# ubisoft/ubisoft-laforge-ZeroEGGS

Measured on AMD Instinct MI355X. Metric: train_frames_per_sec, higher is better.
Workload: dtype f32; 1 GPU; configs_v1.json nets (25.5M params, random-init), batch 32/GPU x 256-frame windows from synthetic 60fps 2-min clips, style example 384 frames, full train step (gather+fwd+loss+bwd+allreduce+RAdam); global_batch=32, window=256, parallelism=dp1

## Files before the change

### include/zeggs_hip.h

```cpp
#ifndef ZEGGS_HIP_H
#define ZEGGS_HIP_H
#include <stddef.h>
#include <stdint.h>

#ifdef __cplusplus
extern "C" {
#endif

int zeggs_version(void);
const char* zeggs_last_error(void);
int zeggs_set_option(const char* name, int value);
int zeggs_timing_ms(int which, float* ms);

int zeggs_gemm(const float* A, const float* B, float* C, const float* bias, int M, int N, int K,
               long sam, long sak, long sbk, long sbn, long scm, long scn, int nbatch, long bsA,
               long bsB, long bsC, float alpha, float beta, int act, void* stream);
int zeggs_gemm_tn_bias(const float* dy, long lddy, const float* x, long ldx, float* dW, long lddw, int M_contract, int N, int K,
                       float beta, float* db, void* stream);
int zeggs_gemm_direct_selftest(int big, int depth, int shield);
int zeggs_gemm_direct_state(int big, int depth, int shield);
int zeggs_gemm_direct_warm(void);
int zeggs_gemm_route(int direct, int shield, int depth, int reserve);
int zeggs_gemm_route_get(int* out4);
int zeggs_gemm_kbatch(const float* A, const float* B, float* C, int M, int N, int K, long sam, long sak, long sbk, long sbn,
// ... 68 lines not shown
                            const ZeggsStyleGrads*, void* ws, size_t ws_bytes, void* stream);
int zeggs_style_encoder_bwd_ex(const ZeggsStyleDims*, const ZeggsStyleParams*, const float* dout,
                               const ZeggsStyleGrads*, void* ws, size_t ws_bytes, void* stream, int grads_zeroed);
int zeggs_style_encoder_bwd_part(const ZeggsStyleDims*, const ZeggsStyleParams*, const float* dout, const ZeggsStyleGrads*, void* ws,
                                 size_t ws_bytes, void* stream, int grads_zeroed, int part);
typedef struct {
  int B, L, C, H, O;
} ZeggsStyleGruDims;
typedef struct {
  const float *c0_w, *c0_b;
  const float *c2_w, *c2_b;
  const float *w_ih, *w_hh, *b_ih, *b_hh;
  const float *w_ih_r, *w_hh_r, *b_ih_r, *b_hh_r;
  const float *p_w, *p_b;
} ZeggsStyleGruParams;
typedef struct {
  float *c0_w, *c0_b, *c2_w, *c2_b, *w_ih, *w_hh, *b_ih, *b_hh, *w_ih_r, *w_hh_r, *b_ih_r, *b_hh_r, *p_w, *p_b;
} ZeggsStyleGruGrads;
size_t zeggs_style_encoder_gru_workspace_bytes(const ZeggsStyleGruDims*);
int zeggs_style_encoder_gru_fwd(const ZeggsStyleGruDims*, const ZeggsStyleGruParams*, const float* x, float* out,
                                void* ws, size_t ws_bytes, void* stream);
int zeggs_style_encoder_gru_bwd(const ZeggsStyleGruDims*, const ZeggsStyleGruParams*, const float* dout,
                                const ZeggsStyleGruGrads*, void* ws, size_t ws_bytes, void* stream);
int zeggs_vae_reparam_fwd(const float* enc, const float* eps, float* z, float* mu_out ,
                          float* logvar_out , int B, int S, float temperature, void* stream);
int zeggs_vae_reparam_bwd(const float* enc, const float* eps, const float* dz, const float* dmu,
                          const float* dlogvar, float* denc, int B, int S, float temperature, void* stream);

typedef struct {
  int B, T, PI, PO, SP, ST, H;
  float dt;
  int film;
} ZeggsDecDims;
typedef struct {
  const float *l0_w, *l0_b;
  const float *w_ih0, *w_hh0, *b_ih0, *b_hh0;
  const float *w_ih1, *w_hh1, *b_ih1, *b_hh1;
  const float *l2_w, *l2_b;
  const float *c0_w, *c0_b, *c1_w, *c1_b, *c2_w, *c2_b;
  const float *l3_w, *l3_b;
  const float *g_w, *g_b, *be_w, *be_b;
} ZeggsDecParams;
typedef struct {
  float *l0_w, *l0_b, *w_ih0, *w_hh0, *b_ih0, *b_hh0, *w_ih1, *w_hh1, *b_ih1, *b_hh1, *l2_w, *l2_b, *c0_w,
      *c0_b, *c1_w, *c1_b, *c2_w, *c2_b, *l3_w, *l3_b, *g_w, *g_b, *be_w, *be_b;
} ZeggsDecGrads;
typedef struct {
  const float *in_mean, *in_std;
  const float *out_mean, *out_std;
} ZeggsDecStats;
size_t zeggs_decoder_workspace_bytes(const ZeggsDecDims*, int training);
int zeggs_decoder_fwd(const ZeggsDecDims*, const ZeggsDecParams*, const ZeggsDecStats*, const float* pose0,
                      const float* rpos0, const float* rrot0, const float* gaze, const float* speech,
                      const float* style, float* pose, float* rpos, float* rrot, int training, void* ws,
                      size_t ws_bytes, void* stream);
int zeggs_decoder_fwd_state(const ZeggsDecDims*, const ZeggsDecParams*, const ZeggsDecStats*, const float* pose0,
                            const float* rpos0, const float* rrot0, const float* gaze, const float* speech,
                            const float* style, float* pose, float* rpos, float* rrot, const float* h_in,
                            float* h_out, void* ws, size_t ws_bytes, void* stream);
int zeggs_persistent_state(int which );
int zeggs_tp_stamps(const ZeggsDecDims*, void* ws, size_t ws_bytes, unsigned long long* out );
int zeggs_tp_waits(const ZeggsDecDims*, void* ws, size_t ws_bytes, unsigned long long* out );
int zeggs_tp_dual_stamps(const ZeggsDecDims*, void* ws, size_t ws_bytes, unsigned long long* out );
int zeggs_bp_stamps(const ZeggsDecDims*, void* ws, size_t ws_bytes, unsigned long long* out );
int zeggs_bp_waits(const ZeggsDecDims*, void* ws, size_t ws_bytes, unsigned long long* out );
int zeggs_decoder_chain_errors(const ZeggsDecDims*, int training, void* ws, size_t ws_bytes, int* out);
int zeggs_decoder_chain_stamps(const ZeggsDecDims*, int training, void* ws, size_t ws_bytes,
                               unsigned long long* out );
int zeggs_decoder_bwd(const ZeggsDecDims*, const ZeggsDecParams*, const ZeggsDecStats*, const float* gaze,
                      const float* pose, const float* rpos, const float* rrot, const float* dpose,
                      const float* drpos, const float* drrot, const ZeggsDecGrads*, float* dspeech,
                      float* dstyle, void* ws, size_t ws_bytes, void* stream);
#define ZEGGS_STATUS_WORDS 4
#define ZEGGS_GAVE_UP_DECODE 1u
#define ZEGGS_GAVE_UP_TRAIN_FWD 2u
#define ZEGGS_GAVE_UP_BPTT 4u
#define ZEGGS_GAVE_UP_BATCH_FWD 8u
typedef struct {
  int prepared;
  int defer_wgrads;
  void* wgrad_stream;
  unsigned* status;
  int grads_zeroed;
} ZeggsDecCall;
int zeggs_decoder_fwd_ex(const ZeggsDecDims*, const ZeggsDecParams*, const ZeggsDecStats*, const float* pose0,
                         const float* rpos0, const float* rrot0, const float* gaze, const float* speech,
                         const float* style, float* pose, float* rpos, float* rrot, int training, void* ws,
                         size_t ws_bytes, void* stream, const ZeggsDecCall* call);
int zeggs_decoder_bwd_ex(const ZeggsDecDims*, const ZeggsDecParams*, const ZeggsDecStats*, const float* gaze,
                         const float* pose, const float* rpos, const float* rrot, const float* dpose,
                         const float* drpos, const float* drrot, const ZeggsDecGrads*, float* dspeech,
                         float* dstyle, void* ws, size_t ws_bytes, void* stream, const ZeggsDecCall* call);
int zeggs_decoder_fwd_state_ex(const ZeggsDecDims*, const ZeggsDecParams*, const ZeggsDecStats*, const float* pose0,
                               const float* rpos0, const float* rrot0, const float* gaze, const float* speech,
                               const float* style, float* pose, float* rpos, float* rrot, const float* h_in,
                               float* h_out, void* ws, size_t ws_bytes, void* stream, const ZeggsDecCall* call);
size_t zeggs_decoder_batch_workspace_bytes(const ZeggsDecDims*);
int zeggs_decoder_batch_prepare(const ZeggsDecDims*, const ZeggsDecParams*, const ZeggsDecStats*, void* ws, size_t ws_bytes,
                                void* stream);
int zeggs_decoder_state_init(const ZeggsDecDims*, const ZeggsDecParams*, const ZeggsDecStats*, const float* pose0,
                             const float* rpos0, const float* rrot0, const float* gaze0, const float* style0, float* h_out,
                             void* ws, size_t ws_bytes, void* stream);
int zeggs_decoder_fwd_batch(const ZeggsDecDims*, const ZeggsDecParams*, const ZeggsDecStats*, const float* pose0,
                            const float* rpos0, const float* rrot0, const float* gaze, const float* speech,
                            const float* style, float* pose, float* rpos, float* rrot, const float* h_in, float* h_out,
                            void* ws, size_t ws_bytes, void* stream, const ZeggsDecCall* call, int mode);
int zeggs_decoder_batch_last_path(void);
int zeggs_decoder_wgrads(const ZeggsDecDims*, const ZeggsDecGrads*, void* ws, size_t ws_bytes, int what, void* stream);
int zeggs_decoder_prepare(const ZeggsDecDims*, const ZeggsDecParams*, const ZeggsDecStats*, void* ws, size_t ws_bytes,
                          void* stream);
int zeggs_side_stream(void** out );

typedef struct {
  int B, T, J, S;
  float dt;
} ZeggsLossDims;
size_t zeggs_loss_workspace_bytes(const ZeggsLossDims*);
int zeggs_loss_fwd_bwd(const ZeggsLossDims*, const int* parents, const float* o_pose, const float* o_rpos,
                       const float* o_rrot, const float* w_pose, const float* w_rpos, const float* w_rrot,
                       const float* gaze, const float* mu, const float* logvar, float kl_weight, float* terms,
                       float* dpose, float* drpos, float* drrot, float* dmu, float* dlogvar, float gscale,
                       void* ws, size_t ws_bytes, void* stream);

int zeggs_loss_prepare_truth(const ZeggsLossDims*, const int* parents, const float* w_pose, const float* w_rpos,
                             const float* w_rrot, const float* gaze, void* ws, size_t ws_bytes, void* stream);
int zeggs_loss_fwd_bwd_ex(const ZeggsLossDims*, const int* parents, const float* o_pose, const float* o_rpos,
                          const float* o_rrot, const float* w_pose, const float* w_rpos, const float* w_rrot,
                          const float* gaze, const float* mu, const float* logvar, float kl_weight, float* terms,
                          float* dpose, float* drpos, float* drrot, float* dmu, float* dlogvar, float gscale,
                          void* ws, size_t ws_bytes, void* stream, int truth_prepared);

#define ZEGGS_EVAL_COLS 22
size_t zeggs_loss_eval_workspace_bytes(const ZeggsLossDims*);
int zeggs_loss_eval(const ZeggsLossDims*, const int* parents, const float* o_pose, const float* o_rpos, const float* o_rrot,
                    const float* w_pose, const float* w_rpos, const float* w_rrot, const float* gaze, const float* mu,
                    const float* logvar, double* rows , void* ws, size_t ws_bytes, void* stream);
int zeggs_eval_accumulate(const double* rows, const int* group , int B, int groups, double* acc, void* stream);
int zeggs_gemm_fixed_order(int on);
enum {
  ZEGGS_GEMM_ROUTE_NONE = 0,
  ZEGGS_GEMM_ROUTE_SKINNY,
  ZEGGS_GEMM_ROUTE_M32_SPLIT,
  ZEGGS_GEMM_ROUTE_M32,
  ZEGGS_GEMM_ROUTE_MID_SPLIT,
  ZEGGS_GEMM_ROUTE_SK_DIRECT,
  ZEGGS_GEMM_ROUTE_SK_BF16_SPLIT,
  ZEGGS_GEMM_ROUTE_SK_DMA,
  ZEGGS_GEMM_ROUTE_SK_LDS_128,
  ZEGGS_GEMM_ROUTE_SK_LDS_256,
  ZEGGS_GEMM_ROUTE_SPLITK,
  ZEGGS_GEMM_ROUTE_HALF,
  ZEGGS_GEMM_ROUTE_TILE_128,
  ZEGGS_GEMM_ROUTE_TILE_64,
  ZEGGS_GEMM_ROUTE_COUNT
};
int zeggs_test_gemm_route_log(int reset, int* last4, long* counts, int ncounts);

int zeggs_radam_step(float* p, const float* g, float* m, float* v, long n, float beta1, float beta2, float eps,
                     float step_scale, int rectified, void* stream);
int zeggs_radam_step_guarded(float* p, const float* g, float* m, float* v, long n, float beta1, float beta2, float eps,
                             float step_scale, int rectified, unsigned* status, const float* gflag, void* stream);
int zeggs_radam_step_guarded_part(float* p, const float* g, float* m, float* v, long n, float beta1, float beta2, float eps,
                                  float step_scale, int rectified, unsigned* status, const float* gflag, int count_skip,
                                  void* stream);
int zeggs_radam_step_wd(float* p, const float* g, float* m, float* v, long n, float beta1, float beta2, float eps,
                        float step_scale, int rectified, float decay, unsigned* status, const float* gflag, int count_skip,
                        void* stream);
int zeggs_radam_step_c(float* p, const float* g, float* m, float* v, long n, float beta1, float beta2, float comp1, float comp2,
                       float eps, float step_scale, int rectified, float decay, unsigned* status, const float* gflag,
                       int count_skip, void* stream);
int zeggs_radam_step_d(float* p, const float* g, float* m, float* v, long n, double beta1, double beta2, double comp1, double comp2,
                       float eps, float step_scale, int rectified, float decay, unsigned* status, const float* gflag,
                       int count_skip, void* stream);
int zeggs_status_flag(const unsigned* status, float* dst , void* stream);
int zeggs_test_cotenant(int workgroups, int threads, float ms, float* scratch, long n, void* stream);
int zeggs_test_attention_fwd(const float* qkv, float* O, float* lse, int B, int L, int E, int NH, float p, uint64_t seed, void* stream);
int zeggs_test_attention_bwd(const float* qkv, const float* O, const float* lse, const float* dO, float* dqkv, float* dsum,
                             float* dbias , int B, int L, int E, int NH, float p, uint64_t seed, void* stream);

int zeggs_gather_windows(const float* frames, int width, const int64_t* starts, int B, int T, float* out,
                         void* stream);
int zeggs_gather_rows(const float* frames, int width, const int64_t* rows, long nrows, float* out, int out_ld,
                      void* stream);

typedef struct {
  int n_fft, hop, n_mels, fs;
  float fps, min_clip;
  double pre_emph;
  int flags;
} ZeggsMelDims;
long zeggs_mel_stft_frames(const ZeggsMelDims*, long n_samples);
size_t zeggs_mel_workspace_bytes(const ZeggsMelDims*, long n_samples);
int zeggs_mel_features(const ZeggsMelDims*, const float* wav, long n_samples, const double* filterbank,
                       int n_frames, float* out, void* ws, size_t ws_bytes, void* stream);
long zeggs_mel_frames_ready(const ZeggsMelDims*, long n_samples);
size_t zeggs_mel_range_workspace_bytes(const ZeggsMelDims*, long k0, long k1);
int zeggs_mel_features_range(const ZeggsMelDims*, const float* wav, long n_samples, int final, const double* filterbank,
                             long k0, long k1, float* out, void* ws, size_t ws_bytes, void* stream);
long zeggs_mel_window_first_sample(const ZeggsMelDims*, long k0);
int zeggs_mel_features_window(const ZeggsMelDims*, const float* wav_window, long base, long n_samples, int final,
                              const double* filterbank, long k0, long k1, float* out, void* ws, size_t ws_bytes, void* stream);
int zeggs_mel_last_form(void);

size_t zeggs_loudness_workspace_bytes(long n_samples, int nblocks, long chunk);
int zeggs_loudness_gain(const float* wav, long n_samples, int rate, double target, const double* coef, const double* trans,
                        long chunk, const long* blk_lo, const long* blk_hi, int nblocks, int f32_stages, double* result,
                        float* gain32, void* ws, size_t ws_bytes, void* stream);

int zeggs_gather_example(const float* frames, int width, const int64_t* rows, int B, int L, const float* mean, const float* stdv,
                         float* out, int out_width, int pad, void* stream);
int zeggs_normalize_rows(float* x, long rows, int width, long ld, const float* mean, const float* stdv,
                         float std_scalar, void* stream);

int zeggs_fill(float* dst, long n, float value, void* stream);
int zeggs_scale_copy(float* dst, const float* src, long n, const float* dev_scale ,
                     float alpha, void* stream);
int zeggs_randn(float* out, long n, uint64_t seed, void* stream);
int zeggs_dropout(float* x, long n, float p, uint64_t seed, void* stream);
int zeggs_broadcast_time(float* out , const float* z , int B, int T, int S, void* stream);
int zeggs_sum_time(float* dz , const float* dout , int B, int T, int S, void* stream);

int zeggs_normalize_vec_fwd(const float* x, float* y, long rows, int width, float eps, void* stream);
int zeggs_normalize_vec_bwd(const float* x, const float* dy, float* dx, long rows, int width, float eps, void* stream);
int zeggs_vectorize_input_fwd(int B, int J, const float* root_pos, const float* root_rot, const float* root_vel,
                              const float* root_vrt, const float* lpos, const float* ltxy, const float* lvel,
                              const float* lvrt, const float* gaze_pos, const float* in_mean, const float* in_std,
                              float* out, void* stream);
int zeggs_vectorize_input_bwd(int B, int J, const float* root_pos, const float* root_rot, const float* gaze_pos,
                              const float* in_std, const float* dout, float* d_root_pos, float* d_root_rot,
                              float* d_root_vel, float* d_root_vrt, float* d_lpos, float* d_ltxy, float* d_lvel,
                              float* d_lvrt, float* d_gaze_pos, void* stream);
int zeggs_devectorize_output_fwd(int B, int J, float dt, const float* predicted, const float* root_pos,
                                 const float* root_rot, const float* out_mean, const float* out_std, float* pose,
                                 float* new_root_pos, float* new_root_rot, void* stream);
int zeggs_devectorize_output_bwd(int B, int J, float dt, const float* predicted, const float* root_pos,
                                 const float* root_rot, const float* out_mean, const float* out_std, const float* d_pose,
                                 const float* d_new_root_pos, const float* d_new_root_rot, float* d_predicted,
                                 float* d_root_pos, float* d_root_rot, void* stream);
int zeggs_kl_div_fwd(const float* mu, const float* logvar, int B, int S, float* out, void* stream);
int zeggs_kl_div_bwd(const float* mu, const float* logvar, int B, int S, const float* dout, float* dmu, float* dlogvar,
                     void* stream);
int zeggs_mask_from_lengths(const int64_t* lengths, int B, int max_len, uint8_t* mask, void* stream);

typedef struct {
  int N, J, hips, spine2, head;
  double dt;
  int order;
} ZeggsAnimDims;
typedef struct {
  double *root_pos, *root_rot, *root_vel, *root_vrt;
  double *lpos, *lrot, *lvel, *lvrt;
  float* ltxy;
  double *cpos, *crot, *cvel, *cvrt;
  float* ctxy;
  double *gaze_pos, *gaze_dir;
} ZeggsAnimOut;
size_t zeggs_anim_features_workspace_bytes(const ZeggsAnimDims*);
int zeggs_anim_features(const ZeggsAnimDims*, const int* parents, const double* euler_deg, const double* positions,
                        const ZeggsAnimOut* out, void* ws, size_t ws_bytes, void* stream);

typedef struct {
  int T, J, rebase;
  double start_pos[3], start_rot[4];
  int order;
} ZeggsBvhDims;
int zeggs_pose_to_bvh(const ZeggsBvhDims*, const float* root_pos, const float* root_rot, const float* lpos,
                      const float* ltxy, double* positions, double* euler_deg, void* stream);

int zeggs_pose_to_bvh_table(const ZeggsBvhDims*, const float* root_pos, const float* root_rot, const float* lpos,
                            const float* ltxy, const float* ref_root_pos, const float* ref_root_rot, const int* seq,
                            double* table, void* stream);

int zeggs_write_table_text(const char* path, int append, const double* table , long rows, int cols);
int zeggs_parse_table_text(const char* text, size_t len, double* table , long rows, int cols);
int zeggs_format_table_text(const double* table , long rows, int cols, char* out, size_t cap, size_t* written);

size_t zeggs_table_text_workspace_bytes(long rows, int cols);
int zeggs_table_text_device(const double* table, long rows, int cols, char* text, size_t cap, long long* row_end,
                            unsigned* status, void* ws, size_t ws_bytes, void* stream);

int zeggs_spline_chunk(int* chunk, int* halo, int* narrow_width);
size_t zeggs_spline_resample_workspace_bytes(long N, int W);
int zeggs_spline_resample(const double* y, long N, int W, long M, double* out, void* ws, size_t ws_bytes, void* stream);
size_t zeggs_rot_stretch_workspace_bytes(long N, int J, long M);
int zeggs_rot_stretch(const double* euler_deg, long N, int J, long M, int order, double* out_deg, void* ws, size_t ws_bytes, void* stream);
int zeggs_audio_prepare(const float* wav, long n_wav, const long* intervals, int n_intervals, long start, long end, float* out_f32,
                        double* out_f64, void* stream);
int zeggs_center_take(double* positions, double* euler_deg, long N, int J, int order, int round_f32, void* ws, size_t ws_bytes,
                      void* stream);
size_t zeggs_masked_stats_workspace_bytes(long R, int D);
int zeggs_masked_stats(const float* x, const unsigned char* mask, long R, int D, double* mean, double* std_, double* pooled, void* ws,
                       size_t ws_bytes, void* stream);

int zeggs_sweep_graph_stats(long* captures, long* replays);

#ifdef __cplusplus
}
#endif
#endif
```

### ubisoft-laforge-zeroeggs_amd/csrc/encoders.hip

```cpp
#include "../../include/zeggs_hip.h"
#include "common.h"
#include "gemm.h"
#include "kernels.h"

namespace {

struct SpeechWs {
  float *h0p, *h1, *wf1, *wb1;
  float *d2, *dh1pp, *dh0p, *dh0, *dwf1;
};

SpeechWs carve_speech(const ZeggsSpeechDims& d, Arena& a) {
  SpeechWs w;
  const long BT = (long)d.B * d.T, pad = d.KW - 1;
  w.h0p = a.f((long)d.B * (d.T + pad) * d.H);
  w.h1 = a.f(BT * d.O);
  w.wf1 = a.f((long)d.KW * d.H * d.O);
  w.wb1 = a.f((long)d.KW * d.O * d.H);
  w.d2 = a.f(BT * d.O);
  w.dh1pp = a.f((long)d.B * (d.T + 2 * pad) * d.O);
  w.dh0p = a.f((long)d.B * (d.T + pad) * d.H);
  w.dh0 = a.f(BT * d.H);
  w.dwf1 = a.f((long)d.KW * d.H * d.O);
  return w;
// ... 130 lines not shown
  w.lse = w.dsum = nullptr;
  if (w.fused) {
    w.P = w.Pd = nullptr;
    w.lse = a.f(B * NH * L); w.dsum = a.f(B * NH * L);
  } else {
    w.P = a.f(B * NH * L * L);
    w.Pd = d.dropout ? a.f(B * NH * L * L) : nullptr;
  }
  w.O = a.f(BL * E);
  w.ao = a.f(BL * E); w.ma = a.f(BL); w.ra = a.f(BL);
  w.ap = a.f(B * LP * E);
  w.f1p = a.f(B * LP * E);
  w.f2 = a.f(BL * E); w.mf = a.f(BL); w.rf = a.f(BL);
  w.f = a.f(BL * E);
  w.S = w.fused ? nullptr : a.f(B * NH * L * L);
  long big = BL * (long)(H > 3 * E ? H : 3 * E);
  const long HE = H > E ? H : E;
  long dw = (long)C * H;
  if ((long)H * E > dw) dw = (long)H * E;
  if ((long)E * E > dw) dw = (long)E * E;
  w.t0 = a.f(B * LP * HE); w.t1 = a.f(big); w.t2 = a.f(big); w.t3 = a.f(B * LP * HE);
  w.dqkv = a.f(BL * 3 * E);
  w.dwf = a.f(3L * dw);
  w.t0a = a.f(B * LP * E); w.t0b = a.f(B * LP * E); w.t1a = a.f(BL * E);
  return w;
}

}

extern "C" size_t zeggs_style_encoder_workspace_bytes(const ZeggsStyleDims* d) {
  Arena a(nullptr, 0);
  carve_style(*d, a);
  return a.off + 256;
}

extern "C" int zeggs_style_encoder_fwd(const ZeggsStyleDims* dp, const ZeggsStyleParams* P, const float* x,
                                       const float* pos, float* out, void* ws, size_t ws_bytes, void* stream) {
  return zeggs_style_encoder_fwd_part(dp, P, x, pos, out, ws, ws_bytes, stream, 3);
}
extern "C" size_t zeggs_style_encoder_input_offset(const ZeggsStyleDims* d) {
  char base[1];
  Arena a(base, ~(size_t)0);
  StyleWs w = carve_style(*d, a);
  return (size_t)((char*)w.xp - base);
}
extern "C" int zeggs_style_encoder_fwd_part(const ZeggsStyleDims* dp, const ZeggsStyleParams* P, const float* x, const float* pos,
                                            float* out, void* ws, size_t ws_bytes, void* stream, int part) {
  const ZeggsStyleDims& d = *dp;
  hipStream_t s = (hipStream_t)stream;
  Arena a(ws, ws_bytes);
  StyleWs w = carve_style(d, a);
  ZCHECK(a.ok(), "style encoder: workspace too small (%zu < %zu)", ws_bytes, a.off);
  ZCHECK(d.E % d.NH == 0, "style encoder: E %% heads != 0");
  const int B = d.B, L = d.L, C = d.C, H = d.H, E = d.E, NH = d.NH, HD = E / NH, LP = L + 2;
  const long BL = (long)B * L;
  const float p2 = d.dropout ? 0.2f : 0.f, p1 = d.dropout ? 0.1f : 0.f;
  const float eps = 1e-5f;
  const bool fuse0 = H <= 512, fuse = E <= 512;
  const RowView c1v = rv(w.c1, L, (long)LP * H), c2v = rv(w.c2, L, (long)LP * E);
  if (part & 1) {
  {
    const PackConvW items[4] = {{w.wf0, nullptr, P->c0_w, H, C, 3}, {w.wf4, w.wb4, P->c4_w, E, H, 3},
                                {w.wff0, w.wfb0, P->ff0_w, E, E, 3}, {w.wff2, w.wfb2, P->ff2_w, E, E, 3}};
    ZTRY(k_pack_conv_w_multi(items, 4, s));
  }
  if (!(part & 4)) ZTRY(k_pad_rows(w.xp, x, B, L, C, 1, 1, 0, s));
  if (fuse0) ZTRY(conv_flat(w.xp, C, w.wf0, 3 * C, H, w.c1, B * LP - 2, s));
  else ZTRY(conv_gemm(w.xp, (long)LP * C, C, w.wf0, 3 * C, H, w.c1, H, (long)LP * H, P->c0_b, B, L, ACT_RELU, s));
  }
  if (!(part & 2)) return 0;
  if (fuse0) {
    LnFwdFused q = ln_fwd_fused_args((int)BL, H, eps);
    q.x = c1v; q.pre_bias = P->c0_b; q.pre_act = ACT_RELU;
    q.y = rv(w.a1p + H, L, (long)LP * H); q.gamma = P->ln0_g; q.beta = P->ln0_b; q.mean = w.m1; q.rstd = w.r1;
    q.p_post = p2; q.seed_post = d.seed + 1; q.pad_L = L;
    ZTRY(k_ln_fwd_fused(q, s));
  } else {
  ZTRY(k_layernorm_fwd_v(rv(w.a1p + H, L, (long)LP * H), c1v, rv(nullptr), P->ln0_g, P->ln0_b, w.m1, w.r1,
                          (int)BL, H, eps, s));
  ZTRY(k_dropout_rows(w.a1p + H, (int)BL, H, H, L, (long)LP * H, p2, d.seed + 1, s));
  ZTRY(k_pad_edges(w.a1p, B, L, H, 1, 1, 0, s));
  }
  if (fuse) ZTRY(conv_flat(w.a1p, H, w.wf4, 3 * H, E, w.c2, B * LP - 2, s));
  else ZTRY(conv_gemm(w.a1p, (long)LP * H, H, w.wf4, 3 * H, E, w.c2, E, (long)LP * E, P->c4_b, B, L, ACT_RELU, s));
  if (fuse) {
    LnFwdFused q = ln_fwd_fused_args((int)BL, E, eps);
    q.x = c2v; q.pre_bias = P->c4_b; q.pre_act = ACT_RELU;
    q.y = rv(w.h); q.gamma = P->ln1_g; q.beta = P->ln1_b; q.mean = w.m2; q.rstd = w.r2;
    q.p_post = p2; q.seed_post = d.seed + 2; q.table = pos; q.table_L = L;
    ZTRY(k_ln_fwd_fused(q, s));
  } else {
  ZTRY(k_layernorm_fwd_v(rv(w.h), c2v, rv(nullptr), P->ln1_g, P->ln1_b, w.m2, w.r2, (int)BL, E, eps, s));
  ZTRY(k_dropout(w.h, BL * E, p2, d.seed + 2, s));
  ZTRY(k_add_rows_bcast(w.h, pos, B, L, E, s));
  }
  ZTRY(gemm_nt(w.h, E, P->in_w, E, w.qkv, 3 * E, P->in_b, (int)BL, 3 * E, E, ACT_NONE, 0.f, s));
  if (w.fused) {
    ZTRY(k_attn_fwd(w.qkv, w.O, w.lse, B, L, E, NH, p1, d.seed + 3, s));
  } else {
  {
    GemmArgs g = gemm_args(w.qkv, w.qkv + E, w.S, L, L, HD);
    g.sam = 3 * E; g.sak = 1; g.sbk = 1; g.sbn = 3 * E; g.scm = L; g.scn = 1;
    g.nb1 = NH; g.bsA0 = (long)L * 3 * E; g.bsA1 = HD; g.bsB0 = (long)L * 3 * E; g.bsB1 = HD;
    g.bsC0 = (long)NH * L * L; g.bsC1 = (long)L * L; g.alpha = 1.0f / sqrtf((float)HD);
    ZTRY(launch_gemm(g, B * NH, s));
  }
  ZTRY(k_softmax_fwd(w.P, w.Pd, w.S, (long)B * NH * L, L, p1, d.seed + 3, s));
  {
    const float* Pm = w.Pd ? w.Pd : w.P;
    GemmArgs g = gemm_args(Pm, w.qkv + 2 * E, w.O, L, HD, L);
    g.sam = L; g.sak = 1; g.sbk = 3 * E; g.sbn = 1; g.scm = E; g.scn = 1;
    g.nb1 = NH; g.bsA0 = (long)NH * L * L; g.bsA1 = (long)L * L; g.bsB0 = (long)L * 3 * E; g.bsB1 = HD;
    g.bsC0 = (long)L * E; g.bsC1 = HD;
    ZTRY(launch_gemm(g, B * NH, s));
  }
  }
  ZTRY(gemm_nt(w.O, E, P->out_w, E, w.ao, E, P->out_b, (int)BL, E, E, ACT_NONE, 0.f, s));
  if (fuse) {
    LnFwdFused q = ln_fwd_fused_args((int)BL, E, eps);
    q.x = rv(w.ao); q.res = rv(w.h); q.y = rv(w.ap + E, L, (long)LP * E); q.gamma = P->lna_g; q.beta = P->lna_b;
    q.mean = w.ma; q.rstd = w.ra; q.p_pre = p1; q.seed_pre = d.seed + 4; q.pad_L = L;
    ZTRY(k_ln_fwd_fused(q, s));
  } else {
  ZTRY(k_dropout(w.ao, BL * E, p1, d.seed + 4, s));
  ZTRY(k_layernorm_fwd_v(rv(w.ap + E, L, (long)LP * E), rv(w.ao), rv(w.h), P->lna_g, P->lna_b, w.ma, w.ra, (int)BL, E,
                          eps, s));
  ZTRY(k_pad_edges(w.ap, B, L, E, 1, 1, 0, s));
  }
  ZTRY(conv_gemm(w.ap, (long)LP * E, E, w.wff0, 3 * E, E, w.f1p + E, E, (long)LP * E, P->ff0_b, B, L, ACT_RELU, s));
  ZTRY(k_pad_edges(w.f1p, B, L, E, 1, 1, 0, s));
  ZTRY(conv_gemm(w.f1p, (long)LP * E, E, w.wff2, 3 * E, E, w.f2, E, (long)L * E, fuse ? nullptr : P->ff2_b, B, L, ACT_NONE, s));
  if (fuse) {
    LnFwdFused q = ln_fwd_fused_args((int)BL, E, eps);
    q.x = rv(w.f2); q.pre_bias = P->ff2_b; q.pre_act = ACT_NONE; q.res = rv(w.ap + E, L, (long)LP * E); q.y = rv(w.f); q.gamma = P->lnf_g; q.beta = P->lnf_b;
    q.mean = w.mf; q.rstd = w.rf; q.p_pre = p1; q.seed_pre = d.seed + 5;
    ZTRY(k_ln_fwd_fused(q, s));
  } else {
  ZTRY(k_dropout(w.f2, BL * E, p1, d.seed + 5, s));
  ZTRY(k_layernorm_fwd_v(rv(w.f), rv(w.f2), rv(w.ap + E, L, (long)LP * E), P->lnf_g, P->lnf_b, w.mf, w.rf, (int)BL, E,
                          eps, s));
  }
  ZTRY(k_meanpool_fwd(out, w.f, B, L, E, s));
  return 0;
}

extern "C" int zeggs_style_encoder_bwd(const ZeggsStyleDims* dp, const ZeggsStyleParams* P, const float* dout,
                                       const ZeggsStyleGrads* G, void* ws, size_t ws_bytes, void* stream) {
  return zeggs_style_encoder_bwd_ex(dp, P, dout, G, ws, ws_bytes, stream, 0);
}
extern "C" int zeggs_style_encoder_bwd_ex(const ZeggsStyleDims* dp, const ZeggsStyleParams* P, const float* dout,
                                          const ZeggsStyleGrads* G, void* ws, size_t ws_bytes, void* stream, int grads_zeroed) {
  return zeggs_style_encoder_bwd_part(dp, P, dout, G, ws, ws_bytes, stream, grads_zeroed, 3);
}
extern "C" int zeggs_style_encoder_bwd_part(const ZeggsStyleDims* dp, const ZeggsStyleParams* P, const float* dout,
                                            const ZeggsStyleGrads* G, void* ws, size_t ws_bytes, void* stream, int grads_zeroed,
                                            int part) {
  ZCHECK(part >= 1 && part <= 3, "style encoder bwd: part must be 1, 2 or 3");
  const bool chain = part & 1, inl = part == 3, only_w = part == 2;
  const ZeggsStyleDims& d = *dp;
  const float gb = grads_zeroed ? 1.f : 0.f;
  hipStream_t s = (hipStream_t)stream;
  Arena a(ws, ws_bytes);
  StyleWs w = carve_style(d, a);
  ZCHECK(a.ok(), "style encoder bwd: workspace too small");
  const int B = d.B, L = d.L, C = d.C, H = d.H, E = d.E, NH = d.NH, HD = E / NH, LP = L + 2;
  const long BL = (long)B * L;
  const float p2 = d.dropout ? 0.2f : 0.f, p1 = d.dropout ? 0.1f : 0.f;
  float *t0 = w.t0, *t1 = w.t1, *t2 = w.t2, *t3 = w.t3;
  float *t0a = w.t0a, *t0b = w.t0b, *t1a = w.t1a;
  auto dw_ff2 = [&](hipStream_t q) -> int {
    ZTRY(conv_dw_gemm(w.f1p, (long)LP * E, E, t0a + E, E, (long)LP * E, w.dwf, 3 * E, E, B, L, q));
    return k_unpack_conv_dw(G->ff2_w, w.dwf, E, E, 3, q);
  };
  auto dw_ff0 = [&](hipStream_t q) -> int {
    ZTRY(conv_dw_gemm(w.ap, (long)LP * E, E, t0b + E, E, (long)LP * E, w.dwf, 3 * E, E, B, L, q));
    return k_unpack_conv_dw(G->ff0_w, w.dwf, E, E, 3, q);
  };
  auto dw_out = [&](hipStream_t q) -> int { return gemm_tn(t1a, E, w.O, E, G->out_w, E, (int)BL, E, E, gb, q); };
  auto dw_in = [&](hipStream_t q) -> int { return gemm_tn(w.dqkv, 3 * E, w.h, E, G->in_w, E, (int)BL, 3 * E, E, gb, q); };
  auto dw_c4 = [&](hipStream_t q) -> int {
    ZTRY(conv_dw_gemm(w.a1p, (long)LP * H, H, t0 + E, E, (long)LP * E, w.dwf, 3 * H, E, B, L, q));
    return k_unpack_conv_dw(G->c4_w, w.dwf, E, H, 3, q);
  };
  auto dw_c0 = [&](hipStream_t q) -> int {
    ZTRY(conv_dw_gemm(w.xp, (long)LP * C, C, t2, H, (long)L * H, w.dwf, 3 * C, H, B, L, q));
    return k_unpack_conv_dw(G->c0_w, w.dwf, H, C, 3, q);
  };
  if (only_w) {
    ZTRY(dw_ff2(s)); ZTRY(dw_ff0(s)); ZTRY(dw_out(s)); ZTRY(dw_in(s)); ZTRY(dw_c4(s)); ZTRY(dw_c0(s));
    return 0;
  }
  (void)chain;
  if (!grads_zeroed) {
    ZTRY(k_fill(G->lnf_g, E, 0.f, s)); ZTRY(k_fill(G->lnf_b, E, 0.f, s)); ZTRY(k_fill(G->ff2_b, E, 0.f, s));
    ZTRY(k_fill(G->ff0_b, E, 0.f, s)); ZTRY(k_fill(G->lna_g, E, 0.f, s)); ZTRY(k_fill(G->lna_b, E, 0.f, s));
    ZTRY(k_fill(G->out_b, E, 0.f, s)); ZTRY(k_fill(G->ln1_g, E, 0.f, s)); ZTRY(k_fill(G->ln1_b, E, 0.f, s));
    ZTRY(k_fill(G->c4_b, E, 0.f, s)); ZTRY(k_fill(G->ln0_g, H, 0.f, s)); ZTRY(k_fill(G->ln0_b, H, 0.f, s));
    ZTRY(k_fill(G->c0_b, H, 0.f, s));
    if (w.fused) ZTRY(k_fill(G->in_b, 3 * E, 0.f, s));
  }
  const RowView t0in = rv(t0 + E, L, (long)LP * E);
  const RowView t0ain = rv(t0a + E, L, (long)LP * E), t0bin = rv(t0b + E, L, (long)LP * E);
  {
    LnBwdFused q = ln_bwd_fused_args((int)BL, E);
    q.dy_pool = dout; q.pool_L = L;
    q.x = rv(w.f2); q.res = rv(w.ap + E, L, (long)LP * E); q.gamma = P->lnf_g; q.mean = w.mf; q.rstd = w.rf;
    q.dgamma = G->lnf_g; q.dbeta = G->lnf_b;
    q.dx_raw = rv(t2); q.out = t0ain; q.pad_L = L; q.p_post = p1; q.seed_post = d.seed + 5; q.dbias = G->ff2_b;
    ZTRY(k_ln_bwd_fused(q, s));
  }
  if (inl) ZTRY(dw_ff2(s));
  ZTRY(conv_gemm(t0a, (long)LP * E, E, w.wfb2, 3 * E, E, t1, E, (long)L * E, nullptr, B, L, ACT_NONE, s));
  {
    LnBwdFused q = ln_bwd_fused_args((int)BL, E);
    q.dyA = rv(t1); q.out = t0bin; q.pad_L = L; q.ysave = rv(w.f1p + E, L, (long)LP * E); q.act = ACT_RELU; q.dbias = G->ff0_b;
    ZTRY(k_ln_bwd_fused(q, s));
  }
  if (inl) ZTRY(dw_ff0(s));
  ZTRY(conv_gemm(t0b, (long)LP * E, E, w.wfb0, 3 * E, E, t1, E, (long)L * E, nullptr, B, L, ACT_NONE, s));
  {
    LnBwdFused q = ln_bwd_fused_args((int)BL, E);
    q.dyA = rv(t2); q.dyB = rv(t1);
    q.x = rv(w.ao); q.res = rv(w.h); q.gamma = P->lna_g; q.mean = w.ma; q.rstd = w.ra; q.dgamma = G->lna_g; q.dbeta = G->lna_b;
    q.dx_raw = rv(t3); q.out = rv(t1a); q.p_post = p1; q.seed_post = d.seed + 4; q.dbias = G->out_b;
    ZTRY(k_ln_bwd_fused(q, s));
  }
  if (inl) ZTRY(dw_out(s));
  ZTRY(gemm_nn(t1a, E, P->out_w, E, t2, E, (int)BL, E, E, 0.f, s));
  if (w.fused) {
    ZTRY(k_attn_bwd(w.qkv, w.O, w.lse, t2, w.dqkv, w.dsum, G->in_b, B, L, E, NH, p1, d.seed + 3, s));
  } else {
  const float* Pm = w.Pd ? w.Pd : w.P;
  {
    GemmArgs g = gemm_args(t2, w.qkv + 2 * E, w.S, L, L, HD);
    g.sam = E; g.sak = 1; g.sbk = 1; g.sbn = 3 * E; g.scm = L; g.scn = 1;
    g.nb1 = NH; g.bsA0 = (long)L * E; g.bsA1 = HD; g.bsB0 = (long)L * 3 * E; g.bsB1 = HD;
    g.bsC0 = (long)NH * L * L; g.bsC1 = (long)L * L;
    ZTRY(launch_gemm(g, B * NH, s));
  }
  {
    GemmArgs g = gemm_args(Pm, t2, w.dqkv + 2 * E, L, HD, L);
    g.sam = 1; g.sak = L; g.sbk = E; g.sbn = 1; g.scm = 3 * E; g.scn = 1;
    g.nb1 = NH; g.bsA0 = (long)NH * L * L; g.bsA1 = (long)L * L; g.bsB0 = (long)L * E; g.bsB1 = HD;
    g.bsC0 = (long)L * 3 * E; g.bsC1 = HD;
    ZTRY(launch_gemm(g, B * NH, s));
  }
  ZTRY(k_softmax_bwd(w.S, w.S, w.P, (long)B * NH * L, L, p1, d.seed + 3, s));
  const float sc = 1.0f / sqrtf((float)HD);
  {
    GemmArgs g = gemm_args(w.S, w.qkv + E, w.dqkv, L, HD, L);
    g.sam = L; g.sak = 1; g.sbk = 3 * E; g.sbn = 1; g.scm = 3 * E; g.scn = 1;
    g.nb1 = NH; g.bsA0 = (long)NH * L * L; g.bsA1 = (long)L * L; g.bsB0 = (long)L * 3 * E; g.bsB1 = HD;
    g.bsC0 = (long)L * 3 * E; g.bsC1 = HD; g.alpha = sc;
    ZTRY(launch_gemm(g, B * NH, s));
  }
  {
    GemmArgs g = gemm_args(w.S, w.qkv, w.dqkv + E, L, HD, L);
    g.sam = 1; g.sak = L; g.sbk = 3 * E; g.sbn = 1; g.scm = 3 * E; g.scn = 1;
    g.nb1 = NH; g.bsA0 = (long)NH * L * L; g.bsA1 = (long)L * L; g.bsB0 = (long)L * 3 * E; g.bsB1 = HD;
    g.bsC0 = (long)L * 3 * E; g.bsC1 = HD; g.alpha = sc;
    ZTRY(launch_gemm(g, B * NH, s));
  }
  }
  if (inl) ZTRY(dw_in(s));
  if (!w.fused) ZTRY(k_colsum(G->in_b, w.dqkv, BL, 3 * E, 3 * E, gb, s));
  ZTRY(gemm_nn(w.dqkv, 3 * E, P->in_w, E, t1, E, (int)BL, 3 * E, E, 0.f, s));
  {
    LnBwdFused q = ln_bwd_fused_args((int)BL, E);
    q.dyA = rv(t1); q.dyB = rv(t3); q.p_pre = p2; q.seed_pre = d.seed + 2;
    q.x = rv(w.c2, L, (long)LP * E); q.gamma = P->ln1_g; q.mean = w.m2; q.rstd = w.r2; q.dgamma = G->ln1_g; q.dbeta = G->ln1_b;
    q.out = t0in; q.pad_L = L; q.ysave = rv(w.c2, L, (long)LP * E); q.act = ACT_RELU; q.dbias = G->c4_b;
    ZTRY(k_ln_bwd_fused(q, s));
  }
  if (inl) ZTRY(dw_c4(s));
  ZTRY(conv_gemm(t0, (long)LP * E, E, w.wb4, 3 * E, H, t1, H, (long)L * H, nullptr, B, L, ACT_NONE, s));
  {
    LnBwdFused q = ln_bwd_fused_args((int)BL, H);
    q.dyA = rv(t1); q.p_pre = p2; q.seed_pre = d.seed + 1;
    q.x = rv(w.c1, L, (long)LP * H); q.gamma = P->ln0_g; q.mean = w.m1; q.rstd = w.r1; q.dgamma = G->ln0_g; q.dbeta = G->ln0_b;
    q.out = rv(t2); q.ysave = rv(w.c1, L, (long)LP * H); q.act = ACT_RELU; q.dbias = G->c0_b;
    ZTRY(k_ln_bwd_fused(q, s));
  }
  if (inl) ZTRY(dw_c0(s));
  return 0;
}
```

### ubisoft-laforge-zeroeggs_amd/csrc/gemm.h

```cpp
#pragma once
#include <hip/hip_runtime.h>

struct GemmArgs {
  const float* A;
  const float* B;
  float* C;
  const float* bias;
  int M, N, K;
  long sam, sak, sbk, sbn, scm, scn;
  long bsA0, bsA1, bsB0, bsB1, bsC0, bsC1;
  int nb1;
  int kbatch;
  long kbsA, kbsB;
  int splitk;
  float alpha, beta;
  int act;
  float* asum;
};

GemmArgs gemm_args(const float* A, const float* B, float* C, int M, int N, int K);
int launch_gemm(GemmArgs g, int nbatch, hipStream_t s, bool* asum_taken = nullptr);
int gemm_nt(const float* x, long ldx, const float* W, long ldw, float* y, long ldy, const float* bias, int M,
            int N, int K, int act, float beta, hipStream_t s);
struct GemmNtItem { const float* x; long ldx; const float* W; long ldw; float* y; long ldy; const float* bias; int N, K, act; };
int gemm_nt_multi(const GemmNtItem* items, int n, int M, hipStream_t s);
int gemm_nn(const float* dy, long lddy, const float* W, long ldw, float* dx, long lddx, int M, int N_contract,
            int K_out, float beta, hipStream_t s);
int gemm_nn_actbwd(const float* dy, long lddy, const float* W, long ldw, float* dx, long lddx, int M, int N_contract,
                   int K_out, float beta, const float* ysave, long ldys, int act, hipStream_t s);
int gemm_tn(const float* dy, long lddy, const float* x, long ldx, float* dW, long lddw, int M_contract, int N,
            int K, float beta, hipStream_t s);
int gemm_tn_bias(const float* dy, long lddy, const float* x, long ldx, float* dW, long lddw, int M_contract, int N,
                 int K, float beta, float* db, hipStream_t s);
```

### ubisoft-laforge-zeroeggs_amd/csrc/gemm.hip

```cpp
#include <type_traits>
#include "common.h"
#include <vector>

#include "gemm.h"
#include "gemm_route.h"
#include "kernels.h"

extern int g_gemm_split_bf16;
bool gemm_split_ok(const GemmArgs& g);
int launch_tn_split(GemmArgs g, hipStream_t s);
bool stream_capturing(hipStream_t s);

int g_gemm_streamk_wgs = 0;
int g_gemm_wg_target = 6144;

namespace {

constexpr int BK = 16;

template <int E>
__device__ __forceinline__ void load_contig(float (&r)[E], const float* p, int nvalid) {
  if (nvalid >= E) {
    if constexpr (E == 16) {
#pragma unroll
// ... 394 lines not shown
    int mo[MT], no[NT];
#pragma unroll
    for (int i = 0; i < MT; ++i) { const int m = m_base + 32 * i + l31; mo[i] = m < g.M ? m : g.M - 1; }
#pragma unroll
    for (int j = 0; j < NT; ++j) { const int n = n_base + 32 * j + l31; no[j] = n < g.N ? n : g.N - 1; }
    unsigned voa[MT], vob[NT];
#pragma unroll
    for (int i = 0; i < MT; ++i) voa[i] = (unsigned)(((long)mo[i] + (long)kh * g.sak) * 4);
#pragma unroll
    for (int j = 0; j < NT; ++j) vob[j] = (unsigned)(((long)no[j] + (long)kh * g.sbk) * 4);
    f16v acc[MT][NT];
#pragma unroll
    for (int i = 0; i < MT; ++i)
#pragma unroll
      for (int j = 0; j < NT; ++j)
#pragma unroll
        for (int e = 0; e < 16; ++e) acc[i][j][e] = 0.f;
    float sa[MT];
#pragma unroll
    for (int i = 0; i < MT; ++i) sa[i] = 0.f;
    int c = c0;
    while (c < c1) {
      const int kb = c / chunks_per_batch, cb = c - kb * chunks_per_batch;
      int ce = c1 - kb * chunks_per_batch;
      ce = ce < chunks_per_batch ? ce : chunks_per_batch;
      const int p0 = cb * CH, p1 = ce * CH < npairs ? ce * CH : npairs, n = p1 - p0;
      const float* Ab = g.A + (long)kb * g.kbsA + (long)(2 * p0) * g.sak;
      const float* Bb = g.B + (long)kb * g.kbsB + (long)(2 * p0) * g.sbk;
      const long a2 = 2 * g.sak, b2 = 2 * g.sbk;
      float ra[D][MT], rb[D][NT];
      auto fetch = [&](int slot, int pair) {
        const unsigned long long ap = (unsigned long long)(Ab + (long)pair * a2), bp = (unsigned long long)(Bb + (long)pair * b2);
        const unsigned alo = __builtin_amdgcn_readfirstlane((unsigned)ap), ahi = __builtin_amdgcn_readfirstlane((unsigned)(ap >> 32));
        const unsigned blo = __builtin_amdgcn_readfirstlane((unsigned)bp), bhi = __builtin_amdgcn_readfirstlane((unsigned)(bp >> 32));
        const unsigned long long as = ((unsigned long long)ahi << 32) | alo, bs = ((unsigned long long)bhi << 32) | blo;
#pragma unroll
        for (int i = 0; i < MT; ++i) asm volatile("global_load_dword %0, %1, %2" : "=v"(ra[slot][i]) : "v"(voa[i]), "s"(as) : "memory");
#pragma unroll
        for (int j = 0; j < NT; ++j) asm volatile("global_load_dword %0, %1, %2" : "=v"(rb[slot][j]) : "v"(vob[j]), "s"(bs) : "memory");
      };
#define ZG_LANDED(S, Y)                                                                                                       \
  do {                                                                                                                         \
    if constexpr (MT == 4)                                                                                                     \
      asm volatile("s_waitcnt vmcnt(%10)\n\tv_add_f32 %6, %6, %0\n\tv_add_f32 %7, %7, %1\n\tv_add_f32 %8, %8, %2\n\tv_add_f32 %9, %9, %3" \
                   : "+v"(ra[S][0]), "+v"(ra[S][1]), "+v"(ra[S][MT > 2 ? 2 : 0]), "+v"(ra[S][MT > 3 ? 3 : 1]),              \
                     "+v"(rb[S][0]), "+v"(rb[S][1]), "+v"(sa[0]), "+v"(sa[1]), "+v"(sa[MT > 2 ? 2 : 0]), "+v"(sa[MT > 3 ? 3 : 1]) \
                   : "n"(Y) : "memory");                                                                                       \
    else                                                                                                                       \
      asm volatile("s_waitcnt vmcnt(%6)\n\tv_add_f32 %4, %4, %0\n\tv_add_f32 %5, %5, %1"                                       \
                   : "+v"(ra[S][0]), "+v"(ra[S][1]), "+v"(rb[S][0]), "+v"(rb[S][1]), "+v"(sa[0]), "+v"(sa[1]) : "n"(Y) : "memory"); \
  } while (0)
      static_assert((MT == 4 || MT == 2) && NT == 2, "direct kernel: wave tiles 128 x 64 and 64 x 64");
      constexpr int LG = MT + NT;
      auto mma = [&](int slot) {
#pragma unroll
        for (int i = 0; i < MT; ++i)
#pragma unroll
          for (int j = 0; j < NT; ++j) acc[i][j] = __builtin_amdgcn_mfma_f32_32x32x2f32(ra[slot][i], rb[slot][j], acc[i][j], 0, 0, 0);
      };
#pragma unroll
      for (int u = 0; u < D; ++u)
        if (u < n) fetch(u, u);
      int p = 0;
      for (; p + 2 * D <= n; p += D) {
#pragma unroll
        for (int u = 0; u < D; ++u) {
          ZG_LANDED(u, (D - 1) * LG);
          mma(u);
          __builtin_amdgcn_sched_barrier(0);
          fetch(u, p + u + D);
          __builtin_amdgcn_sched_barrier(0);
        }
      }
#pragma unroll
      for (int u = 0; u < D; ++u)
        if (p + u < n) ZG_LANDED(u, 0);
#pragma unroll
      for (int u = 0; u < D; ++u)
        if (p + u < n) {
          mma(u);
          if (p + u + D < n) { fetch(u, p + u + D); ZG_LANDED(u, 0); }
        }
      p += D;
#pragma unroll
      for (int u = 0; u < D; ++u)
        if (p + u < n) mma(u);
#undef ZG_LANDED
      c = (kb + 1) * chunks_per_batch < c1 ? (kb + 1) * chunks_per_batch : c1;
    }
#pragma unroll
    for (int i = 0; i < MT; ++i)
#pragma unroll
      for (int j = 0; j < NT; ++j) {
        const int nn = n_base + 32 * j + l31;
        if (nn >= g.N) continue;
#pragma unroll
        for (int e = 0; e < 16; ++e) {
          const int m = m_base + 32 * i + (e & 3) + 8 * (e >> 2) + 4 * kh;
          if (m < g.M) atomicAdd(g.C + (long)m * g.scm + nn, g.alpha * acc[i][j][e]);
        }
      }
    if (g.asum != nullptr && (tile % width) / gsz == 0 && wn == 0) {
#pragma unroll
      for (int i = 0; i < MT; ++i) {
        const float v = sa[i] + __shfl_xor(sa[i], 32, 64);
        const int m = m_base + 32 * i + l31;
        if (kh == 0 && m < g.M) atomicAdd(g.asum + m, g.alpha * v);
      }
    }
    it += c1 - c0;
  }
}
template <int MT, int NT, int D>
__global__ __launch_bounds__(256, 2) void gemm_tn_direct_kernel(GemmArgs g, int tiles_x, int tiles_y, int chunks_per_batch) {
  tn_direct_body<MT, NT, D>(g, tiles_x, tiles_y, chunks_per_batch);
}
template <int MT, int NT, int D>
__global__ __launch_bounds__(256, 1) void gemm_tn_direct_shield_kernel(GemmArgs g, int tiles_x, int tiles_y, int chunks_per_batch) {
  asm volatile("" ::: "v255", "a255");
  tn_direct_body<MT, NT, D>(g, tiles_x, tiles_y, chunks_per_batch);
}
int g_gemm_direct = 1;
int g_gemm_direct_depth = 4;
int g_gemm_direct_shield = 0;
int g_gemm_asum = 1;
int g_gemm_direct_reserve = 0;
int g_gemm_direct_wgs = 0;
static thread_local int tl_route[4] = {-1, -1, -1, -1};
static DirectFirstUse g_direct_first_use;
static TnRoute tn_route() {
  return resolve(tl_route, TnRoute{g_gemm_direct, g_gemm_direct_shield, g_gemm_direct_depth, g_gemm_direct_reserve},
                 g_direct_first_use.disabled.load(std::memory_order_acquire));
}
static TnShape tn_shape(const GemmArgs& g) { return TnShape{g.M, g.N, g.K, g.kbatch, g.sak, g.sbk, g.sam, g.sbn, g.scn}; }
static int device_cus() {
  int dev = 0, ncu = 256;
  if (hipGetDevice(&dev) == hipSuccess) (void)hipDeviceGetAttribute(&ncu, hipDeviceAttributeMultiprocessorCount, dev);
  return ncu;
}
int launch_tn_direct(const GemmArgs& g, const DirectPlan& p, hipStream_t s) {
#define ZG_DIRECT(MT_, D_)                                                                                                    \
  do {                                                                                                                         \
    if (p.shield) hipLaunchKernelGGL((gemm_tn_direct_shield_kernel<MT_, 2, D_>), dim3((unsigned)p.nwg), dim3(256), 0, s, g, p.tx, p.ty, p.cpb); \
    else hipLaunchKernelGGL((gemm_tn_direct_kernel<MT_, 2, D_>), dim3((unsigned)p.nwg), dim3(256), 0, s, g, p.tx, p.ty, p.cpb); \
  } while (0)
  if (p.big) { if (p.depth == 8) ZG_DIRECT(4, 8); else if (p.depth == 6) ZG_DIRECT(4, 6); else ZG_DIRECT(4, 4); }
  else { if (p.depth == 8) ZG_DIRECT(2, 8); else if (p.depth == 6) ZG_DIRECT(2, 6); else ZG_DIRECT(2, 4); }
#undef ZG_DIRECT
  ZLAUNCH_CHECK("gemm_tn_direct");
  return 0;
}

enum GemmRoute { GR_NONE = 0, GR_SKINNY, GR_M32_SPLIT, GR_M32, GR_MID_SPLIT, GR_SK_DIRECT, GR_SK_BF16_SPLIT, GR_SK_DMA, GR_SK_LDS_128,
                 GR_SK_LDS_256, GR_SPLITK, GR_HALF, GR_TILE_128, GR_TILE_64, GR_COUNT };
struct GemmRouteLog { int route, splitk, bm, bn; long count[GR_COUNT]; };
static thread_local GemmRouteLog tl_gemm_log;
static inline void log_route(int route, int splitk, int bm, int bn) {
  tl_gemm_log.route = route; tl_gemm_log.splitk = splitk; tl_gemm_log.bm = bm; tl_gemm_log.bn = bn;
  ++tl_gemm_log.count[route];
}
template <int BM, int BN, int WM, int WN>
int launch_streamk_cfg(GemmArgs g, int ncu, hipStream_t s) {
  const int tx = cdiv(g.N, BN), ty = cdiv(g.M, BM);
  const int kt = cdiv(g.K, BK) * g.kbatch;
  g.splitk = kt;
  constexpr int resident = WM * WN > 4 ? 2 : GEMM_MINB;
  long nwg = (long)ncu * (g_gemm_streamk_wgs > 0 ? g_gemm_streamk_wgs : resident);
  const long total = (long)tx * ty * kt;
  if (nwg > total / 16) nwg = total / 16 > 0 ? total / 16 : 1;
  dim3 grid((unsigned)nwg), block(WM * WN * 64);
  const bool akc = (g.sak == 1), bkc = (g.sbk == 1) && (g.sbn != 1 || g.N == 1);
  if (!akc && g.sam != 1) { zeggs_set_error("gemm: A has no unit stride (sam=%ld sak=%ld)", g.sam, g.sak); return -1; }
  if (!bkc && g.sbn != 1) { zeggs_set_error("gemm: B has no unit stride (sbk=%ld sbn=%ld)", g.sbk, g.sbn); return -1; }
  if (akc && bkc) hipLaunchKernelGGL((gemm_streamk_kernel<BM, BN, WM, WN, true, true>), grid, block, 0, s, g, tx, ty);
  else if (akc && !bkc) hipLaunchKernelGGL((gemm_streamk_kernel<BM, BN, WM, WN, true, false>), grid, block, 0, s, g, tx, ty);
  else if (!akc && bkc) hipLaunchKernelGGL((gemm_streamk_kernel<BM, BN, WM, WN, false, true>), grid, block, 0, s, g, tx, ty);
  else hipLaunchKernelGGL((gemm_streamk_kernel<BM, BN, WM, WN, false, false>), grid, block, 0, s, g, tx, ty);
  ZLAUNCH_CHECK("gemm_streamk");
  return 0;
}
static DirectCheck direct_selftest(const DirectPlan& variant) {
  const bool big = variant.big, shield = variant.shield;
  const int M = big ? 64 * 4 * 2 + 37 : 64 * 2 * 2 + 21, N = 128 + 27, K = 2 * 173;
  const long ldA = M + 3, ldB = N + 5;
  std::vector<float> hA((size_t)K * ldA), hB((size_t)K * ldB), hC((size_t)M * N + M);
  unsigned lcg = 12345u;
  auto rnd = [&]() { lcg = lcg * 1664525u + 1013904223u; return (float)((int)(lcg >> 9) - (1 << 22)) * (1.f / (1 << 22)); };
  for (auto& v : hA) v = rnd();
  for (auto& v : hB) v = rnd();
  hipStream_t st = nullptr;
  float* dA = nullptr;
  auto run = [&]() {
    ZCHECK(hipStreamCreateWithFlags(&st, hipStreamNonBlocking) == hipSuccess, "direct TN GEMM self-test: no stream");
    ZCHECK(hipMalloc(&dA, (hA.size() + hB.size() + hC.size()) * 4) == hipSuccess, "direct TN GEMM self-test: no memory");
    float *dB = dA + hA.size(), *dC = dB + hB.size();
    ZCHECK(hipMemcpyAsync(dA, hA.data(), hA.size() * 4, hipMemcpyHostToDevice, st) == hipSuccess &&
           hipMemcpyAsync(dB, hB.data(), hB.size() * 4, hipMemcpyHostToDevice, st) == hipSuccess &&
           hipMemsetAsync(dC, 0, hC.size() * 4, st) == hipSuccess, "direct TN GEMM self-test: copy failed");
    GemmArgs g = gemm_args(dA, dB, dC, M, N, K);
    g.sam = 1; g.sak = ldA; g.sbk = ldB; g.sbn = 1; g.scm = N; g.scn = 1; g.asum = dC + (size_t)M * N;
    ZTRY(launch_tn_direct(g, direct_grid(variant, tn_shape(g), device_cus(), g_gemm_direct_wgs, 0), st));
    ZCHECK(hipMemcpyAsync(hC.data(), dC, hC.size() * 4, hipMemcpyDeviceToHost, st) == hipSuccess &&
           hipStreamSynchronize(st) == hipSuccess, "direct TN GEMM self-test: copy back failed");
    return 0;
  };
  const bool ran = run() == 0;
  if (dA) (void)hipFree(dA);
  if (st) (void)hipStreamDestroy(st);
  if (!ran) return DirectCheck::UNAVAILABLE;
  const float* hS = hC.data() + (size_t)M * N;
  double worst = 0.0;
  for (int m = 0; m < M; ++m) {
    double sa = 0.0;
    for (int k = 0; k < K; ++k) sa += hA[(size_t)k * ldA + m];
    worst = fmax(worst, fabs(sa - hS[m]));
  }
  for (int m = 0; m < M; m += 3)
    for (int n = 0; n < N; ++n) {
      double acc = 0.0;
      for (int k = 0; k < K; ++k) acc += (double)hA[(size_t)k * ldA + m] * hB[(size_t)k * ldB + n];
      worst = fmax(worst, fabs(acc - hC[(size_t)m * N + n]));
    }
  if (worst < 2e-3) return DirectCheck::AGREES;
  fprintf(stderr, "zeggs: direct TN GEMM self-test (wave tile %s, depth %d%s) is off by %.3g\n", big ? "128x64" : "64x64",
          variant.depth, shield ? ", shield" : "", worst);
  return DirectCheck::MISMATCH;
}
int launch_streamk(GemmArgs g, hipStream_t s, bool* asum_taken) {
  if (gemm_split_ok(g)) { log_route(GR_SK_BF16_SPLIT, 0, 256, 128); return launch_tn_split(g, s); }
  const int ncu = device_cus();
  const DirectPlan plan = direct_plan(tn_route(), tn_shape(g), ncu, g_gemm_direct_wgs);
  if (plan.use && g_direct_first_use.go(plan, [s] { return stream_capturing(s); }, direct_selftest)) {
    if (asum_taken) *asum_taken = g.asum != nullptr;
    log_route(GR_SK_DIRECT, 0, plan.big ? 256 : 128, 128);
    return launch_tn_direct(g, plan, s);
  }
  if (dma_ok(g)) { log_route(GR_SK_DMA, 0, 128, 128); return launch_tn_dma(g, s); }
  if (tn_big_output(g.M, g.N) && g.M >= 512) { log_route(GR_SK_LDS_256, 0, 256, 128); return launch_streamk_cfg<256, 128, 4, 2>(g, ncu, s); }
  log_route(GR_SK_LDS_128, 0, 128, 128);
  return launch_streamk_cfg<128, 128, 2, 2>(g, ncu, s);
}

struct SkinnyArgs {
  const float *x, *W, *bias;
  float* y;
  const float* ysave;
  long ldx, ldw, ldy, ldys;
  int M, N, K, act;
  float beta;
};
template <int NBM, bool WKC>
__device__ __forceinline__ void skinny_body(const SkinnyArgs& a, int bx) {
  __shared__ f4 red[8][NBM][64];
  const int tid = threadIdx.x, lane = tid & 63, wave = tid >> 6, r = lane & 15, g = lane >> 4;
  const int M = a.M, N = a.N, K = a.K;
  const int n0 = bx * 16, nblk = (K + 15) >> 4;
  const int wcol = n0 + r < N ? n0 + r : N - 1;
  const float* wp = WKC ? a.W + (long)wcol * a.ldw + 4 * g : a.W + (long)(4 * g) * a.ldw + wcol;
  const float* xp[NBM];
#pragma unroll
  for (int nb = 0; nb < NBM; ++nb) { const int row = nb * 16 + r; xp[nb] = a.x + (long)(row < M ? row : M - 1) * a.ldx + 4 * g; }
  f4 acc[NBM];
#pragma unroll
  for (int nb = 0; nb < NBM; ++nb) acc[nb] = f4{0.f, 0.f, 0.f, 0.f};
  constexpr int GR = 4;
  float wa[GR][4], xa[GR][NBM][4], wq[GR][4], xq[GR][NBM][4];
  auto load = [&](float (&w)[GR][4], float (&xv)[GR][NBM][4], int i0) {
#pragma unroll
    for (int u = 0; u < GR; ++u) {
      const int kb = wave + 8 * (i0 + u);
      const int nv = kb < nblk ? K - (kb * 16 + 4 * g) : 0;
      if constexpr (WKC) load_contig<4>(w[u], wp + kb * 16, nv);
      else {
#pragma unroll
        for (int j = 0; j < 4; ++j) w[u][j] = j < nv ? wp[(long)(kb * 16 + j) * a.ldw] : 0.f;
      }
#pragma unroll
      for (int nb = 0; nb < NBM; ++nb) load_contig<4>(xv[u][nb], xp[nb] + kb * 16, nv);
    }
  };
  auto comp = [&](const float (&w)[GR][4], const float (&xv)[GR][NBM][4]) {
#pragma unroll
    for (int u = 0; u < GR; ++u)
#pragma unroll
      for (int j = 0; j < 4; ++j)
#pragma unroll
        for (int nb = 0; nb < NBM; ++nb) acc[nb] = __builtin_amdgcn_mfma_f32_16x16x4f32(xv[u][nb][j], w[u][j], acc[nb], 0, 0, 0);
  };
  const int ni = (nblk - wave + 7) / 8;
  load(wa, xa, 0);
  for (int i = 0; i < ni; i += 2 * GR) {
    if (i + GR < ni) load(wq, xq, i + GR);
    comp(wa, xa);
    if (i + 2 * GR < ni) load(wa, xa, i + 2 * GR);
    if (i + GR < ni) comp(wq, xq);
  }
#pragma unroll
  for (int nb = 0; nb < NBM; ++nb) red[wave][nb][lane] = acc[nb];
  __syncthreads();
  if (tid < NBM * 64) {
    const int nb = tid >> 6, l = tid & 63;
    f4 sum = red[0][nb][l];
#pragma unroll
    for (int w = 1; w < 8; ++w) sum += red[w][nb][l];
    const int col = n0 + (l & 15);
    if (col < N) {
      const float bv = a.bias ? a.bias[col] : 0.f;
#pragma unroll
      for (int q = 0; q < 4; ++q) {
        const int row = nb * 16 + 4 * (l >> 4) + q;
        if (row < M) {
          float* yp = a.y + (long)row * a.ldy + col;
          float v = sum[q] + bv;
          if (a.beta != 0.f) v += a.beta * *yp;
          if (a.ysave) {
            const float ys = a.ysave[(long)row * a.ldys + col];
            v = a.act == ACT_ELU ? v * d_elu_grad_from_out(ys) : a.act == ACT_RELU ? (ys > 0.f ? v : 0.f) : v;
          } else v = d_act(v, a.act);
          *yp = v;
        }
      }
    }
  }
}
template <int NBM, bool WKC>
__global__ __launch_bounds__(512) void skinny_k(SkinnyArgs a) {
  skinny_body<NBM, WKC>(a, blockIdx.x);
}
struct SkinnyMulti { SkinnyArgs p[3]; int nb[3]; };
template <int NBM, bool WKC>
__global__ __launch_bounds__(512) void skinny_multi_k(SkinnyMulti m) {
  int bx = blockIdx.x;
  if (bx < m.nb[0]) { skinny_body<NBM, WKC>(m.p[0], bx); return; }
  bx -= m.nb[0];
  if (bx < m.nb[1]) { skinny_body<NBM, WKC>(m.p[1], bx); return; }
  skinny_body<NBM, WKC>(m.p[2], bx - m.nb[1]);
}

int launch_skinny(const SkinnyArgs& a, bool wkc, hipStream_t s) {
  const int nbm = cdiv(a.M, 16);
  dim3 grid(cdiv(a.N, 16)), block(512);
#define ZEGGS_SKINNY(NB)                                                             \
  do {                                                                               \
    if (wkc) hipLaunchKernelGGL((skinny_k<NB, true>), grid, block, 0, s, a);         \
    else hipLaunchKernelGGL((skinny_k<NB, false>), grid, block, 0, s, a);            \
  } while (0)
  if (nbm == 1) ZEGGS_SKINNY(1);
  else if (nbm == 2) ZEGGS_SKINNY(2);
  else if (nbm == 3) ZEGGS_SKINNY(3);
  else ZEGGS_SKINNY(4);
#undef ZEGGS_SKINNY
  ZLAUNCH_CHECK("gemm_skinny");
  return 0;
}
bool skinny_ok(const GemmArgs& g, int nbatch) {
  return g.M <= 64 && nbatch == 1 && g.kbatch == 1 && g.sak == 1 && g.scn == 1 && g.alpha == 1.f && g.N >= 64 && g.K >= 64 &&
         ((g.sbk == 1 && g.sbn != 1) || g.sbn == 1) && (g.beta == 0.f || (g.bias == nullptr && g.act == ACT_NONE));
}
SkinnyArgs skinny_args(const GemmArgs& g) {
  SkinnyArgs a;
  memset(&a, 0, sizeof(a));
  a.x = g.A; a.ldx = g.sam; a.W = g.B; a.y = g.C; a.ldy = g.scm; a.bias = g.bias; a.M = g.M; a.N = g.N; a.K = g.K;
  a.act = g.act; a.beta = g.beta;
  a.ldw = (g.sbk == 1 && g.sbn != 1) ? g.sbn : g.sbk;
  return a;
}

}

void zeggs_gemm_set_dma(int on) { g_gemm_dma = on; }
void zeggs_gemm_set_direct(int mode, int wgs) { if (mode >= 0) g_gemm_direct = mode; if (wgs >= 0) g_gemm_direct_wgs = wgs; }
void zeggs_gemm_set_direct_depth(int d) { g_gemm_direct_depth = d; }
void zeggs_gemm_set_direct_shield(int on) { g_gemm_direct_shield = on; }
void zeggs_gemm_set_direct_reserve(int n) { g_gemm_direct_reserve = n; }
extern "C" int zeggs_gemm_route(int direct, int shield, int depth, int reserve) {
  const int r[4] = {direct, shield, depth, reserve};
  memcpy(tl_route, r, sizeof(r));
  return 0;
}
extern "C" int zeggs_gemm_route_get(int* out4) {
  const TnRoute r = tn_route();
  out4[0] = r.direct; out4[1] = r.shield; out4[2] = r.depth; out4[3] = r.reserve;
  return 0;
}
void zeggs_gemm_set_asum(int on) { g_gemm_asum = on; }
int g_gemm_skinny = 1;
int g_gemm_streamk = 1;
int g_gemm_mid_split = 1;
static thread_local int t_gemm_fixed_order = 0;
extern "C" int zeggs_gemm_fixed_order(int on) {
  const int prev = t_gemm_fixed_order;
  t_gemm_fixed_order = on != 0;
  return prev;
}

constexpr long SK_MIN_KTILES = 80;
int launch_gemm(GemmArgs g, int nbatch, hipStream_t s, bool* asum_taken) {
  if (asum_taken) *asum_taken = false;
  if (g.M <= 0 || g.N <= 0 || nbatch <= 0) return 0;
  if (g.nb1 <= 0) g.nb1 = 1;
  if (g.kbatch <= 0) g.kbatch = 1;
  g.splitk = 1;
  const bool may_split = !t_gemm_fixed_order;
  if (g_gemm_skinny && skinny_ok(g, nbatch)) {
    log_route(GR_SKINNY, 1, 16 * (cdiv(g.M, 16) < 4 ? cdiv(g.M, 16) : 4), 16);
    return launch_skinny(skinny_args(g), g.sbk == 1 && g.sbn != 1, s);
  }
  if (g.M <= 32) {
    const long tiles = (long)cdiv(g.N, 128) * nbatch;
    const long ktiles = (long)cdiv(g.K, 16) * g.kbatch;
    const bool plain_beta = g.beta == 0.f || (g.beta == 1.f && g.bias == nullptr && g.act == ACT_NONE);
    if (may_split && nbatch == 1 && g.scn == 1 && plain_beta && ktiles >= 16 && tiles < 128) {
      long sk = (256 + tiles - 1) / tiles;
      if (sk > ktiles / 4) sk = ktiles / 4;
      if (sk > 64) sk = 64;
      if (sk > 1) {
        const float* bias = g.bias;
        const int act = g.act;
        const long n = (long)g.M * g.N, blocks = (n + 255) / 256;
        if (g.beta == 0.f) {
          hipLaunchKernelGGL(rows_fill_k, dim3((unsigned)(blocks > 1024 ? 1024 : blocks)), dim3(256), 0, s, g.C, g.M, g.N, g.scm);
          ZLAUNCH_CHECK("gemm_rows_fill");
        }
        g.bias = nullptr; g.act = ACT_NONE; g.splitk = (int)sk;
        log_route(GR_M32_SPLIT, g.splitk, 32, 128);
        ZTRY((launch_cfg<32, 128, 1, 4>(g, nbatch, s)));
        if (bias || act != ACT_NONE) {
          hipLaunchKernelGGL(rows_bias_act_k, dim3((unsigned)(blocks > 1024 ? 1024 : blocks)), dim3(256), 0, s, g.C, bias, g.M,
                             g.N, g.scm, act);
          ZLAUNCH_CHECK("gemm_rows_bias_act");
        }
        return 0;
      }
    }
    log_route(GR_M32, 1, 32, 128);
    return launch_cfg<32, 128, 1, 4>(g, nbatch, s);
  }
  const bool big = g.M > 64 && g.N > 64;
  const long tiles = big ? (long)cdiv(g.M, 128) * cdiv(g.N, 128) * nbatch : (long)cdiv(g.M, 64) * cdiv(g.N, 64) * nbatch;
  const long ktiles = (long)cdiv(g.K, 16) * g.kbatch;
  {
    const bool flat_c = g.nb1 == 1 && g.scn == 1 && (nbatch == 1 || g.bsC0 == (long)g.M * g.scm);
    const bool plain_beta = g.beta == 0.f || (g.beta == 1.f && g.bias == nullptr && g.act == ACT_NONE);
    const long tiles64 = (long)cdiv(g.M, 64) * cdiv(g.N, 64) * nbatch;
    const bool streamk_case = g_gemm_streamk && nbatch == 1 && g.bias == nullptr && g.act == ACT_NONE && g.scm == g.N && big &&
                              ktiles >= SK_MIN_KTILES && tiles < 1024 * 3;
    if (may_split && g_gemm_mid_split && flat_c && plain_beta && !streamk_case && tiles64 >= 32 && tiles64 < 768 && ktiles >= 16) {
      long sk = (1024 + tiles64 - 1) / tiles64;
      if (sk > ktiles / 6) sk = ktiles / 6;
      if (sk > 8) sk = 8;
      if (sk > 1) {
        const float* bias = g.bias;
        const int act = g.act;
        const int rows = nbatch * g.M;
        const long n = (long)rows * g.N, blocks = (n + 255) / 256;
        if (g.beta == 0.f) {
          hipLaunchKernelGGL(rows_fill_k, dim3((unsigned)(blocks > 2048 ? 2048 : blocks)), dim3(256), 0, s, g.C, rows, g.N, g.scm);
          ZLAUNCH_CHECK("gemm_rows_fill");
        }
        g.bias = nullptr; g.act = ACT_NONE; g.splitk = (int)sk;
        log_route(GR_MID_SPLIT, g.splitk, 64, 64);
        ZTRY((launch_cfg<64, 64, 2, 2>(g, nbatch, s)));
        if (bias || act != ACT_NONE) {
          hipLaunchKernelGGL(rows_bias_act_k, dim3((unsigned)(blocks > 2048 ? 2048 : blocks)), dim3(256), 0, s, g.C, bias, rows,
                             g.N, g.scm, act);
          ZLAUNCH_CHECK("gemm_rows_bias_act");
        }
        return 0;
      }
    }
  }
  const bool can_split = nbatch == 1 && (g.beta == 0.f || g.beta == 1.f) && g.bias == nullptr && g.act == ACT_NONE &&
                         g.scn == 1 && g.scm == g.N && ktiles >= 64;
  if (may_split && g_gemm_streamk && can_split && big && g.nb1 == 1 && tiles < 1024 * 3 && ktiles >= SK_MIN_KTILES) {
    if (g.beta == 0.f) ZTRY(k_fill(g.C, (long)g.M * g.N, 0.f, s));
    return launch_streamk(g, s, asum_taken);
  }
  if (may_split && tiles < g_gemm_wg_target * 5 / 6 && can_split) {
    long sk = (g_gemm_wg_target + tiles - 1) / tiles;
    if (sk > ktiles / 16) sk = ktiles / 16;
    if (sk > 32) sk = 32;
    if (sk > 1) {
      g.splitk = (int)sk;
      if (g.beta == 0.f) ZTRY(k_fill(g.C, (long)g.M * g.N, 0.f, s));
    }
  }
  constexpr bool HALF_TILES = true;
  if (HALF_TILES && big && g.splitk == 1 && tiles > 256 && tiles < 512 && g.N % 64 == 0) {
    log_route(GR_HALF, 1, 128, 64);
    return launch_cfg<128, 64, 2, 2>(g, nbatch, s);
  }
  if (big && (tiles * g.splitk >= 128 || g.splitk > 1)) {
    log_route(g.splitk > 1 ? GR_SPLITK : GR_TILE_128, g.splitk, 128, 128);
    return launch_cfg<128, 128, 2, 2>(g, nbatch, s);
  }
  log_route(g.splitk > 1 ? GR_SPLITK : GR_TILE_64, g.splitk, 64, 64);
  return launch_cfg<64, 64, 2, 2>(g, nbatch, s);
}

extern "C" int zeggs_test_gemm_route_log(int reset, int* last4, long* counts, int ncounts) {
  if (last4) { last4[0] = tl_gemm_log.route; last4[1] = tl_gemm_log.splitk; last4[2] = tl_gemm_log.bm; last4[3] = tl_gemm_log.bn; }
  for (int i = 0; counts && i < ncounts; ++i) counts[i] = i < GR_COUNT ? tl_gemm_log.count[i] : 0;
  if (reset) tl_gemm_log = GemmRouteLog{};
  return GR_COUNT;
}

GemmArgs gemm_args(const float* A, const float* B, float* C, int M, int N, int K) {
  GemmArgs g;
  memset(&g, 0, sizeof(g));
  g.A = A; g.B = B; g.C = C; g.M = M; g.N = N; g.K = K;
  g.nb1 = 1; g.kbatch = 1; g.splitk = 1; g.alpha = 1.f; g.beta = 0.f; g.act = ACT_NONE;
  return g;
}

int gemm_nt(const float* x, long ldx, const float* W, long ldw, float* y, long ldy, const float* bias,
            int M, int N, int K, int act, float beta, hipStream_t s) {
  GemmArgs g = gemm_args(x, W, y, M, N, K);
  g.sam = ldx; g.sak = 1; g.sbk = 1; g.sbn = ldw; g.scm = ldy; g.scn = 1;
  g.bias = bias; g.act = act; g.beta = beta;
  return launch_gemm(g, 1, s);
}
int gemm_nt_multi(const GemmNtItem* it, int n, int M, hipStream_t s) {
  bool one = g_gemm_skinny && n >= 2 && n <= 3 && M <= 64;
  GemmArgs g[3];
  for (int i = 0; i < n && i < 3; ++i) {
    g[i] = gemm_args(it[i].x, it[i].W, it[i].y, M, it[i].N, it[i].K);
    g[i].sam = it[i].ldx; g[i].sak = 1; g[i].sbk = 1; g[i].sbn = it[i].ldw; g[i].scm = it[i].ldy; g[i].scn = 1;
    g[i].bias = it[i].bias; g[i].act = it[i].act;
    one = one && skinny_ok(g[i], 1);
  }
  if (!one) {
    for (int i = 0; i < n; ++i)
      ZTRY(gemm_nt(it[i].x, it[i].ldx, it[i].W, it[i].ldw, it[i].y, it[i].ldy, it[i].bias, M, it[i].N, it[i].K, it[i].act, 0.f, s));
    return 0;
  }
  SkinnyMulti m;
  memset(&m, 0, sizeof(m));
  int total = 0;
  for (int i = 0; i < n; ++i) { m.p[i] = skinny_args(g[i]); m.nb[i] = cdiv(it[i].N, 16); total += m.nb[i]; }
  const int nbm = cdiv(M, 16);
  dim3 grid(total), block(512);
  if (nbm == 1) hipLaunchKernelGGL((skinny_multi_k<1, true>), grid, block, 0, s, m);
  else if (nbm == 2) hipLaunchKernelGGL((skinny_multi_k<2, true>), grid, block, 0, s, m);
  else if (nbm == 3) hipLaunchKernelGGL((skinny_multi_k<3, true>), grid, block, 0, s, m);
  else hipLaunchKernelGGL((skinny_multi_k<4, true>), grid, block, 0, s, m);
  ZLAUNCH_CHECK("gemm_skinny_multi");
  return 0;
}
int gemm_nn(const float* dy, long lddy, const float* W, long ldw, float* dx, long lddx, int M, int N_contract,
            int K_out, float beta, hipStream_t s) {
  GemmArgs g = gemm_args(dy, W, dx, M, K_out, N_contract);
  g.sam = lddy; g.sak = 1; g.sbk = ldw; g.sbn = 1; g.scm = lddx; g.scn = 1; g.beta = beta;
  return launch_gemm(g, 1, s);
}
int gemm_nn_actbwd(const float* dy, long lddy, const float* W, long ldw, float* dx, long lddx, int M, int N_contract,
                   int K_out, float beta, const float* ysave, long ldys, int act, hipStream_t s) {
  GemmArgs g = gemm_args(dy, W, dx, M, K_out, N_contract);
  g.sam = lddy; g.sak = 1; g.sbk = ldw; g.sbn = 1; g.scm = lddx; g.scn = 1; g.beta = beta;
  if (g_gemm_skinny && skinny_ok(g, 1)) {
    SkinnyArgs a = skinny_args(g);
    a.ysave = ysave; a.ldys = ldys; a.act = act;
    return launch_skinny(a, false, s);
  }
  ZTRY(launch_gemm(g, 1, s));
  if (lddx != K_out || ldys != K_out) { zeggs_set_error("gemm_nn_actbwd: strided rows need the one-launch kernel (M <= 64)"); return -1; }
  return k_act_bwd(dx, dx, ysave, (long)M * K_out, act, 1.f, s);
}
int gemm_tn(const float* dy, long lddy, const float* x, long ldx, float* dW, long lddw, int M_contract, int N,
            int K, float beta, hipStream_t s) {
  GemmArgs g = gemm_args(dy, x, dW, N, K, M_contract);
  g.sam = 1; g.sak = lddy; g.sbk = ldx; g.sbn = 1; g.scm = lddw; g.scn = 1; g.beta = beta;
  return launch_gemm(g, 1, s);
}

int gemm_tn_bias(const float* dy, long lddy, const float* x, long ldx, float* dW, long lddw, int M_contract, int N,
                 int K, float beta, float* db, hipStream_t s) {
  GemmArgs g = gemm_args(dy, x, dW, N, K, M_contract);
  g.sam = 1; g.sak = lddy; g.sbk = ldx; g.sbn = 1; g.scm = lddw; g.scn = 1; g.beta = beta;
  g.asum = (beta == 1.f && g_gemm_asum && !g_gemm_split_bf16) ? db : nullptr;
  bool asum_taken = false;
  ZTRY(launch_gemm(g, 1, s, &asum_taken));
  if (!asum_taken) ZTRY(k_colsum(db, dy, M_contract, N, lddy, beta, s));
  return 0;
}

extern "C" int zeggs_gemm_direct_selftest(int big, int depth, int shield) {
  return direct_selftest(direct_variant(big != 0, depth, shield != 0)) == DirectCheck::AGREES ? 1 : 0;
}
extern "C" int zeggs_gemm_direct_state(int big, int depth, int shield) {
  return g_direct_first_use.at(big != 0, depth, shield != 0).load(std::memory_order_acquire);
}
extern "C" int zeggs_gemm_direct_warm(void) {
  const TnRoute r = tn_route();
  bool unavailable = false;
  for (int big = 0; big < 2; ++big)
    for (int shield = 0; shield < 2; ++shield) {
      if (!route_selects(r, big, shield)) continue;
      g_direct_first_use.go(direct_variant(big, r.depth, shield), [] { return false; }, [&](const DirectPlan& v) {
        const DirectCheck c = direct_selftest(v);
        unavailable |= c == DirectCheck::UNAVAILABLE;
        return c;
      });
    }
  return unavailable ? -1 : 0;
}
extern "C" int zeggs_gemm_tn_bias(const float* dy, long lddy, const float* x, long ldx, float* dW, long lddw, int M_contract, int N,
                                  int K, float beta, float* db, void* stream) {
  return gemm_tn_bias(dy, lddy, x, ldx, dW, lddw, M_contract, N, K, beta, db, (hipStream_t)stream);
}

extern "C" int zeggs_gemm(const float* A, const float* B, float* C, const float* bias, int M, int N, int K,
                          long sam, long sak, long sbk, long sbn, long scm, long scn, int nbatch, long bsA,
                          long bsB, long bsC, float alpha, float beta, int act, void* stream) {
  GemmArgs g = gemm_args(A, B, C, M, N, K);
  g.sam = sam; g.sak = sak; g.sbk = sbk; g.sbn = sbn; g.scm = scm; g.scn = scn;
  g.bsA0 = bsA; g.bsB0 = bsB; g.bsC0 = bsC; g.nb1 = 1;
  g.bias = bias; g.alpha = alpha; g.beta = beta; g.act = act;
  return launch_gemm(g, nbatch, (hipStream_t)stream);
}

extern "C" int zeggs_gemm_kbatch(const float* A, const float* B, float* C, int M, int N, int K, long sam, long sak, long sbk,
                                 long sbn, long scm, long scn, int kbatch, long kbsA, long kbsB, float beta, void* stream) {
  GemmArgs g = gemm_args(A, B, C, M, N, K);
  g.sam = sam; g.sak = sak; g.sbk = sbk; g.sbn = sbn; g.scm = scm; g.scn = scn;
  g.kbatch = kbatch; g.kbsA = kbsA; g.kbsB = kbsB; g.beta = beta;
  return launch_gemm(g, 1, (hipStream_t)stream);
}
```

### ubisoft-laforge-zeroeggs_amd/csrc/kernels.h

```cpp
#pragma once
#include <hip/hip_runtime.h>
#include <stdint.h>

struct RowView {
  float* p;
  long rpb, bstride;
};
inline RowView rv(const float* p) { return RowView{(float*)p, 0, 0}; }
inline RowView rv(const float* p, long rpb, long bstride) { return RowView{(float*)p, rpb, bstride}; }
int k_layernorm_fwd_v(RowView y, RowView x, RowView res, const float* gamma, const float* beta, float* mean,
                      float* rstd, int R, int C, float eps, hipStream_t s);
int k_layernorm_bwd_v(RowView dx, RowView dy, RowView x, RowView res, const float* gamma, const float* mean,
                      const float* rstd, float* dgamma, float* dbeta, int R, int C, hipStream_t s);
int k_act_bwd_v(RowView dx, RowView dy, RowView y, long R, int C, int act, float y_scale, hipStream_t s);
struct LnBwdFused {
  RowView dyA, dyB;
  const float* dy_pool;
  int pool_L;
  float p_pre, p_post;
  uint64_t seed_pre, seed_post;
  RowView x, res;
  const float *gamma, *mean, *rstd;
  RowView dx_raw, out, ysave;
  int act, pad_L;
  float *dgamma, *dbeta, *dbias;
  int R, C;
};
LnBwdFused ln_bwd_fused_args(int R, int C);
struct LnFwdFused {
  RowView x, res, y;
  const float* pre_bias;
  int pre_act;
  const float *gamma, *beta, *table;
  float *mean, *rstd;
  float p_pre, p_post, eps;
  uint64_t seed_pre, seed_post;
  int table_L, pad_L, R, C;
};
LnFwdFused ln_fwd_fused_args(int R, int C, float eps);
int k_ln_fwd_fused(const LnFwdFused& a, hipStream_t s);
int k_ln_bwd_fused(const LnBwdFused& a, hipStream_t s);
int k_colsum_v(float* out, RowView x, long R, int C, float beta, hipStream_t s);

int k_fill(float* p, long n, float v, hipStream_t s);
int k_copy(float* dst, const float* src, long n, hipStream_t s);
int k_add_inplace(float* dst, const float* src, long n, hipStream_t s);
int k_act_bwd(float* dx, const float* dy, const float* y, long n, int act, float y_scale, hipStream_t s);
int k_dropout(float* x, long n, float p, uint64_t seed, hipStream_t s);
int k_dropout_rows(float* x, int rows, int cols, long ld, long batch_rows, long batch_stride, float p,
                   uint64_t seed, hipStream_t s);
int k_layernorm_fwd(float* y, const float* x, const float* res, const float* gamma, const float* beta,
                    float* mean, float* rstd, int R, int C, float eps, hipStream_t s);
int k_layernorm_bwd(float* dx, const float* dy, const float* x, const float* res, const float* gamma,
                    const float* mean, const float* rstd, float* dgamma, float* dbeta, int R, int C,
                    hipStream_t s);
int k_softmax_fwd(float* P, float* Pd, const float* S, long R, int L, float p, uint64_t seed, hipStream_t s);
int k_softmax_bwd(float* dS, const float* dPd, const float* P, long R, int L, float p, uint64_t seed,
                  hipStream_t s);
int k_colsum(float* out, const float* x, long R, int C, long ld, float beta, hipStream_t s);
int k_pad_rows(float* dst, const float* src, int B, int T, int C, int pl, int pr, int mode, hipStream_t s);
int k_pad_edges(float* buf, int B, int T, int C, int pl, int pr, int mode, hipStream_t s);
int k_unpad_fold(float* dx, const float* dpad, int B, int T, int C, int pl, int pr, int mode, hipStream_t s);
int k_pack_conv_w(float* wf, float* wb, const float* w, int Co, int Ci, int Kw, hipStream_t s);
struct PackConvW { float *wf, *wb; const float* w; int Co, Ci, Kw; };
int k_pack_conv_w_multi(const PackConvW* items, int n, hipStream_t s);
int k_unpack_conv_dw(float* dw, const float* dwf, int Co, int Ci, int Kw, hipStream_t s);
int k_add_rows_bcast(float* h, const float* table, int B, int L, int C, hipStream_t s);
int k_meanpool_fwd(float* out, const float* f, int B, int L, int C, hipStream_t s);
int k_meanpool_bwd(float* df, const float* dout, int B, int L, int C, hipStream_t s);

int attn_fused_supported(int E, int NH);
int k_attn_fwd(const float* qkv, float* O, float* lse, int B, int L, int E, int NH, float p, uint64_t seed, hipStream_t s);
int k_attn_bwd(const float* qkv, const float* O, const float* lse, const float* dO, float* dqkv, float* dsum, float* dbias,
               int B, int L, int E, int NH, float p, uint64_t seed, hipStream_t s);

struct Arena;
struct SgFast {
  float *pw, *pb, *xf, *Hxf, *DIxf, *DHxf, *GT, *DHn;
  long xf_floats;
  int NB, nT5, nTH, KBH, KB3H;
};
int sg_fast_supported(int B, int H);
SgFast sg_fast_carve(int B, int H, int L, Arena& a);
int sg_fast_fwd(int B, int H, int L, const float* w_hh, const float* b_hh, const float* GI, float* Hs, const SgFast& f,
                hipStream_t s);
int sg_fast_bwd(int B, int H, int L, const float* w_hh, const float* Hs, float* DI, float* dhc, const SgFast& f, hipStream_t s);
```

### ubisoft-laforge-zeroeggs_amd/csrc/kernels.hip

```cpp
#include "common.h"
#include "kernels.h"

namespace {

inline int grid1d(long n, int block = 256) {
  long g = (n + block - 1) / block;
  return (int)(g > 8192 ? 8192 : (g < 1 ? 1 : g));
}
#define GS_LOOP(i, n) for (long i = (long)blockIdx.x * blockDim.x + threadIdx.x; i < (n); i += (long)gridDim.x * blockDim.x)

__device__ __forceinline__ float* rv_row(const RowView& v, long r, int C) {
  if (v.rpb == 0) return v.p + r * C;
  const long b = r / v.rpb;
  return v.p + b * v.bstride + (r - b * v.rpb) * C;
}

__global__ void fill_k(float* p, long n, float v) { GS_LOOP(i, n) p[i] = v; }
__global__ void fill4_k(f4* p, long n4, float v) { const f4 vv = f4{v, v, v, v}; GS_LOOP(i, n4) p[i] = vv; }
__global__ void copy_k(float* d, const float* s, long n) { GS_LOOP(i, n) d[i] = s[i]; }
__global__ void add_k(float* d, const float* s, long n) { GS_LOOP(i, n) d[i] += s[i]; }

__global__ void act_bwd_k(float* dx, const float* dy, const float* y, long n, int act, float ys) {
  GS_LOOP(i, n) {
    float yv = y[i] * ys, g = dy[i];
// ... 438 lines not shown
  float z = 0.f;
  for (int c = lane; c < L; c += 64) z += expf(s[c] - m);
  z = wave_sum(z);
  for (int c = lane; c < L; c += 64) {
    float v = expf(s[c] - m) / z;
    P[row * L + c] = v;
    if (Pd) Pd[row * L + c] = v * dropout_scale(seed, (uint64_t)(row * L + c), p);
  }
}

__global__ __launch_bounds__(256) void softmax_bwd_k(float* dS, const float* dPd, const float* P, long R, int L,
                                                      float p, uint64_t seed) {
  long row = (long)blockIdx.x * 4 + (threadIdx.x >> 6);
  int lane = threadIdx.x & 63;
  if (row >= R) return;
  float acc = 0.f;
  for (int c = lane; c < L; c += 64) {
    long i = row * L + c;
    acc += dPd[i] * dropout_scale(seed, (uint64_t)i, p) * P[i];
  }
  acc = wave_sum(acc);
  for (int c = lane; c < L; c += 64) {
    long i = row * L + c;
    dS[i] = P[i] * (dPd[i] * dropout_scale(seed, (uint64_t)i, p) - acc);
  }
}

__global__ __launch_bounds__(256) void colsum_k(float* out, const float* x, long R, int C, long ld,
                                                 long rows_per_block) {
  __shared__ float red[4][64];
  int cl = threadIdx.x & 63, ph = threadIdx.x >> 6;
  int c = blockIdx.x * 64 + cl;
  long r0 = (long)blockIdx.y * rows_per_block, r1 = r0 + rows_per_block;
  if (r1 > R) r1 = R;
  float s = 0.f;
  if (c < C)
    for (long r = r0 + ph; r < r1; r += 4) s += x[r * ld + c];
  red[ph][cl] = s;
  __syncthreads();
  if (ph == 0 && c < C) atomicAdd(out + c, red[0][cl] + red[1][cl] + red[2][cl] + red[3][cl]);
}

__global__ __launch_bounds__(256) void colsum4_k(float* out, const float* x, long R, int C, long ld, long rows_per_block) {
  __shared__ f4 red[4][64];
  const int cl = threadIdx.x & 63, ph = threadIdx.x >> 6;
  const int c = (blockIdx.x * 64 + cl) * 4;
  const long r0 = (long)blockIdx.y * rows_per_block;
  long r1 = r0 + rows_per_block;
  if (r1 > R) r1 = R;
  f4 s = f4{0.f, 0.f, 0.f, 0.f};
  if (c < C)
    for (long r = r0 + ph; r < r1; r += 4) s += *(const f4*)(x + r * ld + c);
  red[ph][cl] = s;
  __syncthreads();
  if (ph == 0 && c < C) {
    const f4 t = red[0][cl] + red[1][cl] + red[2][cl] + red[3][cl];
    atomicAdd(out + c, t[0]); atomicAdd(out + c + 1, t[1]); atomicAdd(out + c + 2, t[2]); atomicAdd(out + c + 3, t[3]);
  }
}

__global__ __launch_bounds__(256) void colsum_v_k(float* out, RowView x, long R, int C, long rows_per_block) {
  __shared__ float red[4][64];
  int cl = threadIdx.x & 63, ph = threadIdx.x >> 6;
  int c = blockIdx.x * 64 + cl;
  long r0 = (long)blockIdx.y * rows_per_block, r1 = r0 + rows_per_block;
  if (r1 > R) r1 = R;
  float s = 0.f;
  if (c < C)
    for (long r = r0 + ph; r < r1; r += 4) s += rv_row(x, r, C)[c];
  red[ph][cl] = s;
  __syncthreads();
  if (ph == 0 && c < C) atomicAdd(out + c, red[0][cl] + red[1][cl] + red[2][cl] + red[3][cl]);
}

__global__ void scale_k(float* p, long n, float v) { GS_LOOP(i, n) p[i] *= v; }

__global__ void pad_rows_k(float* dst, const float* src, int B, int T, int C, int pl, int pr, int mode) {
  int TP = pl + T + pr;
  long n = (long)B * TP * C;
  GS_LOOP(i, n) {
    int c = (int)(i % C);
    long r = i / C;
    int tp = (int)(r % TP);
    long b = r / TP;
    int t = tp - pl;
    float v = 0.f;
    if (t >= 0 && t < T) v = src[(b * T + t) * C + c];
    else if (mode == 1) v = src[(b * T + (t < 0 ? 0 : T - 1)) * C + c];
    dst[i] = v;
  }
}

__global__ void pad_edges_k(float* buf, int B, int T, int C, int pl, int pr, int mode) {
  int TP = pl + T + pr, NE = pl + pr;
  long n = (long)B * NE * C;
  GS_LOOP(i, n) {
    int c = (int)(i % C);
    long r = i / C;
    int e = (int)(r % NE);
    long b = r / NE;
    int tp = e < pl ? e : T + e;
    int src_t = e < pl ? pl : pl + T - 1;
    float v = mode == 1 ? buf[(b * TP + src_t) * C + c] : 0.f;
    buf[(b * TP + tp) * C + c] = v;
  }
}

__global__ void unpad_fold_k(float* dx, const float* dpad, int B, int T, int C, int pl, int pr, int mode) {
  int TP = pl + T + pr;
  long n = (long)B * T * C;
  GS_LOOP(i, n) {
    int c = (int)(i % C);
    long r = i / C;
    int t = (int)(r % T);
    long b = r / T;
    const float* d = dpad + (b * TP) * C + c;
    float v = d[(long)(t + pl) * C];
    if (mode == 1) {
      if (t == 0) for (int q = 0; q < pl; ++q) v += d[(long)q * C];
      if (t == T - 1) for (int q = 0; q < pr; ++q) v += d[(long)(pl + T + q) * C];
    }
    dx[i] = v;
  }
}

__global__ void pack_conv_w_k(float* wf, float* wb, const float* w, int Co, int Ci, int Kw) {
  long n = (long)Co * Ci * Kw;
  GS_LOOP(i, n) {
    int j = (int)(i % Kw);
    long r = i / Kw;
    int ci = (int)(r % Ci), co = (int)(r / Ci);
    float v = w[i];
    wf[((long)j * Ci + ci) * Co + co] = v;
    if (wb) wb[((long)(Kw - 1 - j) * Co + co) * Ci + ci] = v;
  }
}

struct PackConvW4 { PackConvW it[4]; long end[4]; int n; };
__global__ void pack_conv_w_multi_k(PackConvW4 q) {
  GS_LOOP(g, q.end[q.n - 1]) {
    int k = 0;
    while (g >= q.end[k]) ++k;
    const PackConvW& p = q.it[k];
    const long i = g - (k ? q.end[k - 1] : 0);
    const int j = (int)(i % p.Kw);
    const long r = i / p.Kw;
    const int ci = (int)(r % p.Ci), co = (int)(r / p.Ci);
    const float v = p.w[i];
    p.wf[((long)j * p.Ci + ci) * p.Co + co] = v;
    if (p.wb) p.wb[((long)(p.Kw - 1 - j) * p.Co + co) * p.Ci + ci] = v;
  }
}

__global__ __launch_bounds__(256) void unpack_conv_dw_t_k(float* dw, const float* dwf, int Co, int Ci, int Kw) {
  __shared__ float t[4][32][33];
  const int ci0 = blockIdx.x * 32, co0 = blockIdx.y * 32, tx = threadIdx.x & 31, ty = threadIdx.x >> 5;
  for (int j = 0; j < Kw; ++j)
    for (int r = ty; r < 32; r += 8) {
      const int ci = ci0 + r, co = co0 + tx;
      t[j][r][tx] = (ci < Ci && co < Co) ? dwf[((long)j * Ci + ci) * Co + co] : 0.f;
    }
  __syncthreads();
  const int run = 32 * Kw;
  for (int r = ty; r < 32; r += 8) {
    const int co = co0 + r;
    if (co >= Co) continue;
    for (int e = tx; e < run; e += 32) {
      const int cl = e / Kw, j = e - cl * Kw, ci = ci0 + cl;
      if (ci < Ci) dw[((long)co * Ci + ci) * Kw + j] = t[j][cl][r];
    }
  }
}

__global__ void unpack_conv_dw_k(float* dw, const float* dwf, int Co, int Ci, int Kw) {
  long n = (long)Co * Ci * Kw;
  GS_LOOP(i, n) {
    int j = (int)(i % Kw);
    long r = i / Kw;
    int ci = (int)(r % Ci), co = (int)(r / Ci);
    dw[i] = dwf[((long)j * Ci + ci) * Co + co];
  }
}

__global__ void add_rows_bcast_k(float* h, const float* table, int B, int L, int C) {
  long n = (long)B * L * C, lc = (long)L * C;
  GS_LOOP(i, n) h[i] += table[i % lc];
}

__global__ void meanpool_fwd_k(float* out, const float* f, int B, int L, int C) {
  __shared__ float red[16][64];
  int cl = threadIdx.x & 63, ph = threadIdx.x >> 6;
  int b = blockIdx.y, c = blockIdx.x * 64 + cl;
  float s = 0.f;
  if (c < C)
    for (int l = ph; l < L; l += 16) s += f[((long)b * L + l) * C + c];
  red[ph][cl] = s;
  __syncthreads();
  if (ph == 0 && c < C) {
    float t = 0.f;
#pragma unroll
    for (int q = 0; q < 16; ++q) t += red[q][cl];
    out[(long)b * C + c] = t / (float)L;
  }
}

__global__ void meanpool_bwd_k(float* df, const float* dout, int B, int L, int C) {
  long n = (long)B * L * C;
  GS_LOOP(i, n) {
    int c = (int)(i % C);
    long b = i / ((long)L * C);
    df[i] = dout[b * C + c] / (float)L;
  }
}

}

#define L1D(kernel, n, s, ...)                                                        \
  do {                                                                                \
    if ((n) > 0) {                                                                    \
      hipLaunchKernelGGL(kernel, dim3(grid1d(n)), dim3(256), 0, s, __VA_ARGS__);      \
      ZLAUNCH_CHECK(#kernel);                                                         \
    }                                                                                 \
  } while (0)

int k_fill(float* p, long n, float v, hipStream_t s) {
  const long head = (((size_t)p & 15) && n > 0) ? ((16 - ((size_t)p & 15)) / 4 < (size_t)n ? (long)((16 - ((size_t)p & 15)) / 4) : n) : 0;
  const long n4 = (n - head) / 4, tail = n - head - 4 * n4;
  if (n4 < 1024) { L1D(fill_k, n, s, p, n, v); return 0; }
  if (head) L1D(fill_k, head, s, p, head, v);
  L1D(fill4_k, n4, s, (f4*)(p + head), n4, v);
  if (tail) L1D(fill_k, tail, s, p + head + 4 * n4, tail, v);
  return 0;
}
int k_copy(float* d, const float* src, long n, hipStream_t s) { L1D(copy_k, n, s, d, src, n); return 0; }
int k_add_inplace(float* d, const float* src, long n, hipStream_t s) { L1D(add_k, n, s, d, src, n); return 0; }
int k_act_bwd(float* dx, const float* dy, const float* y, long n, int act, float ys, hipStream_t s) {
  L1D(act_bwd_k, n, s, dx, dy, y, n, act, ys);
  return 0;
}
int k_dropout(float* x, long n, float p, uint64_t seed, hipStream_t s) {
  if (p <= 0.f) return 0;
  L1D(dropout_k, n, s, x, n, p, seed);
  return 0;
}
int k_dropout_rows(float* x, int rows, int cols, long ld, long batch_rows, long batch_stride, float p,
                   uint64_t seed, hipStream_t s) {
  if (p <= 0.f) return 0;
  long n = (long)rows * cols;
  L1D(dropout_rows_k, n, s, x, rows, cols, ld, batch_rows, batch_stride, p, seed);
  return 0;
}
int k_layernorm_fwd_v(RowView y, RowView x, RowView res, const float* gamma, const float* beta, float* mean,
                      float* rstd, int R, int C, float eps, hipStream_t s) {
  hipLaunchKernelGGL(layernorm_fwd_k, dim3(cdiv(R, 4)), dim3(256), 0, s, y, x, res, gamma, beta, mean, rstd, R, C, eps);
  ZLAUNCH_CHECK("layernorm_fwd");
  return 0;
}
int k_layernorm_fwd(float* y, const float* x, const float* res, const float* gamma, const float* beta,
                    float* mean, float* rstd, int R, int C, float eps, hipStream_t s) {
  return k_layernorm_fwd_v(rv(y), rv(x), rv(res), gamma, beta, mean, rstd, R, C, eps, s);
}
int k_layernorm_bwd_v(RowView dx, RowView dy, RowView x, RowView res, const float* gamma, const float* mean,
                      const float* rstd, float* dgamma, float* dbeta, int R, int C, hipStream_t s) {
  const int rpb = 16;
  ZCHECK(C <= 512, "layernorm_bwd: C=%d > 512 unsupported", C);
  if (C <= 128)
    hipLaunchKernelGGL((layernorm_bwd_k<2>), dim3(cdiv(R, rpb)), dim3(256), 0, s, dx, dy, x, res, gamma, mean, rstd,
                       dgamma, dbeta, R, C, rpb);
  else
    hipLaunchKernelGGL((layernorm_bwd_k<8>), dim3(cdiv(R, rpb)), dim3(256), 0, s, dx, dy, x, res, gamma, mean, rstd,
                       dgamma, dbeta, R, C, rpb);
  ZLAUNCH_CHECK("layernorm_bwd");
  return 0;
}
LnFwdFused ln_fwd_fused_args(int R, int C, float eps) {
  LnFwdFused a;
  memset(&a, 0, sizeof(a));
  a.R = R; a.C = C; a.eps = eps; a.table_L = 1;
  return a;
}
static bool rv_al16_(const RowView& v) { return v.p == nullptr || ((((size_t)v.p) & 15) == 0 && (v.rpb == 0 || v.bstride % 4 == 0)); }
extern int g_ln_bwd4;
int k_ln_fwd_fused(const LnFwdFused& a, hipStream_t s) {
  ZCHECK(a.C <= 512, "ln_fwd_fused: C=%d > 512 unsupported", a.C);
  if (g_ln_bwd4 && a.C % 4 == 0 && a.R > 0 && rv_al16_(a.x) && rv_al16_(a.res) && rv_al16_(a.y) && (long)a.R * a.C < (1L << 31)) {
    if (a.C <= 128) hipLaunchKernelGGL((ln_fwd_fused4_k<32, 1>), dim3(cdiv(a.R, 8)), dim3(256), 0, s, a);
    else if (a.C <= 256) hipLaunchKernelGGL((ln_fwd_fused4_k<64, 1>), dim3(cdiv(a.R, 4)), dim3(256), 0, s, a);
    else hipLaunchKernelGGL((ln_fwd_fused4_k<64, 2>), dim3(cdiv(a.R, 4)), dim3(256), 0, s, a);
    ZLAUNCH_CHECK("ln_fwd_fused4");
    return 0;
  }
  if (a.C <= 128) hipLaunchKernelGGL((ln_fwd_fused_k<2>), dim3(cdiv(a.R, 4)), dim3(256), 0, s, a);
  else hipLaunchKernelGGL((ln_fwd_fused_k<8>), dim3(cdiv(a.R, 4)), dim3(256), 0, s, a);
  ZLAUNCH_CHECK("ln_fwd_fused");
  return 0;
}
LnBwdFused ln_bwd_fused_args(int R, int C) {
  LnBwdFused a;
  memset(&a, 0, sizeof(a));
  a.R = R; a.C = C; a.pool_L = 1;
  return a;
}
int g_ln_bwd4 = 1;
static bool rv_al16(const RowView& v) { return v.p == nullptr || ((((size_t)v.p) & 15) == 0 && (v.rpb == 0 || v.bstride % 4 == 0)); }
int k_ln_bwd_fused(const LnBwdFused& a, hipStream_t s) {
  ZCHECK(a.C <= 1024, "ln_bwd_fused: C=%d > 1024 unsupported", a.C);
  ZCHECK(a.out.p != nullptr && (a.dy_pool != nullptr || a.dyA.p != nullptr), "ln_bwd_fused: missing operand");
  const bool al = a.C % 4 == 0 && rv_al16(a.dyA) && rv_al16(a.dyB) && rv_al16(a.x) && rv_al16(a.res) && rv_al16(a.dx_raw) &&
                  rv_al16(a.out) && rv_al16(a.ysave) && (((size_t)a.dy_pool) & 15) == 0 &&
                  a.R > 0 && (long)a.R * a.C < (1L << 31);
  if (g_ln_bwd4 && al && a.C <= 512) {
    auto rows_per_block = [&](int rpp, int blocks) { const int per = cdiv(a.R, blocks); return cdiv(per, rpp) * rpp; };
    if (a.C <= 128 && g_ln_bwd4 == 2) { const int rpb = rows_per_block(8, 512); hipLaunchKernelGGL((ln_bwd_fused4_k<32, 1, 4>), dim3(cdiv(a.R, rpb)), dim3(256), 0, s, a, rpb); }
    else if (a.C <= 128) { const int rpb = rows_per_block(32, 256); hipLaunchKernelGGL((ln_bwd_fused4_k<32, 1, 16>), dim3(cdiv(a.R, rpb)), dim3(1024), 0, s, a, rpb); }
    else if (a.C <= 256) { const int rpb = rows_per_block(8, 256); hipLaunchKernelGGL((ln_bwd_fused4_k<64, 1, 8>), dim3(cdiv(a.R, rpb)), dim3(512), 0, s, a, rpb); }
    else { const int rpb = rows_per_block(4, 512); hipLaunchKernelGGL((ln_bwd_fused4_k<64, 2, 4>), dim3(cdiv(a.R, rpb)), dim3(256), 0, s, a, rpb); }
    ZLAUNCH_CHECK("ln_bwd_fused4");
    return 0;
  }
  const int rpb = 16;
  if (a.C <= 128) hipLaunchKernelGGL((ln_bwd_fused_k<2>), dim3(cdiv(a.R, rpb)), dim3(256), 0, s, a, rpb);
  else if (a.C <= 512) hipLaunchKernelGGL((ln_bwd_fused_k<8>), dim3(cdiv(a.R, rpb)), dim3(256), 0, s, a, rpb);
  else hipLaunchKernelGGL((ln_bwd_fused_k<16>), dim3(cdiv(a.R, rpb)), dim3(256), 0, s, a, rpb);
  ZLAUNCH_CHECK("ln_bwd_fused");
  return 0;
}
int k_layernorm_bwd(float* dx, const float* dy, const float* x, const float* res, const float* gamma,
                    const float* mean, const float* rstd, float* dgamma, float* dbeta, int R, int C,
                    hipStream_t s) {
  return k_layernorm_bwd_v(rv(dx), rv(dy), rv(x), rv(res), gamma, mean, rstd, dgamma, dbeta, R, C, s);
}
int k_act_bwd_v(RowView dx, RowView dy, RowView y, long R, int C, int act, float ys, hipStream_t s) {
  long n = R * C;
  L1D(act_bwd_v_k, n, s, dx, dy, y, R, C, act, ys);
  return 0;
}
int k_colsum_v(float* out, RowView x, long R, int C, float beta, hipStream_t s) {
  if (beta == 0.f) { ZTRY(k_fill(out, C, 0.f, s)); }
  long rpb = 256;
  dim3 grid(cdiv(C, 64), cdiv(R, rpb));
  hipLaunchKernelGGL(colsum_v_k, grid, dim3(256), 0, s, out, x, R, C, rpb);
  ZLAUNCH_CHECK("colsum_v");
  return 0;
}
int k_softmax_fwd(float* P, float* Pd, const float* S, long R, int L, float p, uint64_t seed, hipStream_t s) {
  hipLaunchKernelGGL(softmax_fwd_k, dim3(cdiv(R, 4)), dim3(256), 0, s, P, Pd, S, R, L, p, seed);
  ZLAUNCH_CHECK("softmax_fwd");
  return 0;
}
int k_softmax_bwd(float* dS, const float* dPd, const float* P, long R, int L, float p, uint64_t seed,
                  hipStream_t s) {
  hipLaunchKernelGGL(softmax_bwd_k, dim3(cdiv(R, 4)), dim3(256), 0, s, dS, dPd, P, R, L, p, seed);
  ZLAUNCH_CHECK("softmax_bwd");
  return 0;
}
int k_colsum(float* out, const float* x, long R, int C, long ld, float beta, hipStream_t s) {
  if (beta == 0.f) { ZTRY(k_fill(out, C, 0.f, s)); }
  else if (beta != 1.f) { L1D(scale_k, (long)C, s, out, (long)C, beta); }
  long rpb = 256;
  if (C % 4 == 0 && ld % 4 == 0 && ((uintptr_t)x & 15) == 0 && C >= 256) {
    rpb = 128;
    dim3 grid(cdiv(C, 256), cdiv(R, rpb));
    hipLaunchKernelGGL(colsum4_k, grid, dim3(256), 0, s, out, x, R, C, ld, rpb);
  } else {
    dim3 grid(cdiv(C, 64), cdiv(R, rpb));
    hipLaunchKernelGGL(colsum_k, grid, dim3(256), 0, s, out, x, R, C, ld, rpb);
  }
  ZLAUNCH_CHECK("colsum");
  return 0;
}
int k_pad_rows(float* dst, const float* src, int B, int T, int C, int pl, int pr, int mode, hipStream_t s) {
  long n = (long)B * (pl + T + pr) * C;
  L1D(pad_rows_k, n, s, dst, src, B, T, C, pl, pr, mode);
  return 0;
}
int k_pad_edges(float* buf, int B, int T, int C, int pl, int pr, int mode, hipStream_t s) {
  long n = (long)B * (pl + pr) * C;
  L1D(pad_edges_k, n, s, buf, B, T, C, pl, pr, mode);
  return 0;
}
int k_unpad_fold(float* dx, const float* dpad, int B, int T, int C, int pl, int pr, int mode, hipStream_t s) {
  long n = (long)B * T * C;
  L1D(unpad_fold_k, n, s, dx, dpad, B, T, C, pl, pr, mode);
  return 0;
}
int k_pack_conv_w(float* wf, float* wb, const float* w, int Co, int Ci, int Kw, hipStream_t s) {
  long n = (long)Co * Ci * Kw;
  L1D(pack_conv_w_k, n, s, wf, wb, w, Co, Ci, Kw);
  return 0;
}
int k_pack_conv_w_multi(const PackConvW* items, int n, hipStream_t s) {
  ZCHECK(n >= 1 && n <= 4, "pack_conv_w_multi: %d items", n);
  PackConvW4 q;
  memset(&q, 0, sizeof(q));
  long tot = 0;
  for (int k = 0; k < n; ++k) { q.it[k] = items[k]; tot += (long)items[k].Co * items[k].Ci * items[k].Kw; q.end[k] = tot; }
  q.n = n;
  L1D(pack_conv_w_multi_k, tot, s, q);
  return 0;
}
int k_unpack_conv_dw(float* dw, const float* dwf, int Co, int Ci, int Kw, hipStream_t s) {
  long n = (long)Co * Ci * Kw;
  if (Kw <= 4 && n >= 65536) {
    hipLaunchKernelGGL(unpack_conv_dw_t_k, dim3(cdiv(Ci, 32), cdiv(Co, 32)), dim3(256), 0, s, dw, dwf, Co, Ci, Kw);
    ZLAUNCH_CHECK("unpack_conv_dw_t");
    return 0;
  }
  L1D(unpack_conv_dw_k, n, s, dw, dwf, Co, Ci, Kw);
  return 0;
}
int k_add_rows_bcast(float* h, const float* table, int B, int L, int C, hipStream_t s) {
  long n = (long)B * L * C;
  L1D(add_rows_bcast_k, n, s, h, table, B, L, C);
  return 0;
}
int k_meanpool_fwd(float* out, const float* f, int B, int L, int C, hipStream_t s) {
  hipLaunchKernelGGL(meanpool_fwd_k, dim3(cdiv(C, 64), B), dim3(1024), 0, s, out, f, B, L, C);
  ZLAUNCH_CHECK("meanpool_fwd");
  return 0;
}
int k_meanpool_bwd(float* df, const float* dout, int B, int L, int C, hipStream_t s) {
  long n = (long)B * L * C;
  L1D(meanpool_bwd_k, n, s, df, dout, B, L, C);
  return 0;
}
```

### ubisoft-laforge-zeroeggs_amd/csrc/options.hip

```cpp
#include "../../include/zeggs_hip.h"
#include "common.h"
#include "decoder_ws.h"

extern int g_attn_bwd_one_launch, g_fused_attention;
extern int g_decoder_fast, g_bwd_chunks, g_tp_prologue, g_wgrad_order;
extern int g_stage_variant, g_timing, g_chain, g_sweep_graphs, g_launch_window;
extern int g_tp_tiles4, g_tp_dual;
extern int g_gemm_wg_target, g_gemm_streamk_wgs, g_gemm_mid_split, g_gemm_skinny, g_gemm_streamk, g_gemm_split_bf16;
extern int g_text_emit, g_text_passes;
extern int g_mel_mfma, g_mel_fft, g_mel_exact_log, g_loss_lds, g_ln_bwd4;
void zeggs_gemm_set_dma(int on), zeggs_gemm_set_direct(int mode, int wgs), zeggs_gemm_set_direct_depth(int d);
void zeggs_gemm_set_direct_shield(int on), zeggs_gemm_set_direct_reserve(int n), zeggs_gemm_set_asum(int on);

namespace {
enum Kind { AS_GIVEN, NONZERO, MIN0, MIN1, CALL };
struct Option { const char* name; int* target; Kind kind; int (*set)(int); };
int set_chain(int v) {
#ifndef ZEGGS_CHAIN
  if (v) { zeggs_set_error("option chain: the chained (run-ahead) stage launches lost to the persistent decode kernel and are "
                           "compiled in measurement builds only (-DZEGGS_CHAIN)"); return -1; }
#endif
  g_chain = v;
  return 0;
}
const Option k_options[] = {
  {"attn_bwd_one_launch", &g_attn_bwd_one_launch, NONZERO},
  {"decoder_fast", &g_decoder_fast, AS_GIVEN},
  {"stage_variant", &g_stage_variant, AS_GIVEN},
  {"gemm_wg_target", &g_gemm_wg_target, AS_GIVEN},
  {"timing", &g_timing, AS_GIVEN},
  {"chain", nullptr, CALL, set_chain},
  {"sweep_graphs", &g_sweep_graphs, NONZERO},
  {"launch_window", &g_launch_window, MIN0},
  {"train_persistent", nullptr, CALL, [](int v) { g_sweep_kernels[SWEEP_ROLLOUT].set_enabled(v); return 0; }},
  {"bwd_persistent", nullptr, CALL, [](int v) { g_sweep_kernels[SWEEP_BPTT].set_enabled(v); return 0; }},
  {"persistent", nullptr, CALL, [](int v) { g_sweep_kernels[SWEEP_DECODE].set_enabled(v); return 0; }},
  {"mel_mfma", &g_mel_mfma, NONZERO},
  {"mel_fft", &g_mel_fft, NONZERO},
  {"gemm_streamk_wgs", &g_gemm_streamk_wgs, AS_GIVEN},
  {"gemm_mid_split", &g_gemm_mid_split, NONZERO},
  {"gemm_dma", nullptr, CALL, [](int v) { zeggs_gemm_set_dma(v != 0); return 0; }},
  {"gemm_direct", nullptr, CALL, [](int v) { zeggs_gemm_set_direct(v, -1); return 0; }},
  {"gemm_direct_wgs", nullptr, CALL, [](int v) { zeggs_gemm_set_direct(-1, v); return 0; }},
  {"gemm_direct_depth", nullptr, CALL, [](int v) { zeggs_gemm_set_direct_depth(v); return 0; }},
  {"gemm_direct_shield", nullptr, CALL, [](int v) { zeggs_gemm_set_direct_shield(v); return 0; }},
  {"gemm_direct_reserve", nullptr, CALL, [](int v) { zeggs_gemm_set_direct_reserve(v); return 0; }},
  {"gemm_asum", nullptr, CALL, [](int v) { zeggs_gemm_set_asum(v); return 0; }},
  {"gemm_skinny", &g_gemm_skinny, NONZERO},
  {"gemm_streamk", &g_gemm_streamk, NONZERO},
  {"fused_attention", &g_fused_attention, NONZERO},
  {"bwd_chunks", &g_bwd_chunks, MIN1},
  {"tp_tiles4", &g_tp_tiles4, NONZERO},
  {"tp_dual", &g_tp_dual, NONZERO},
  {"tp_prologue", &g_tp_prologue, NONZERO},
  {"loss_lds", &g_loss_lds, NONZERO},
  {"wgrad_order", &g_wgrad_order, AS_GIVEN},
  {"gemm_split_bf16", nullptr, CALL, [](int v) { g_gemm_split_bf16 = (v == 3 || v == 6 || v == 9) ? v : 0; return 0; }},
  {"poll_stagger", &g_poll_stagger, MIN0},
  {"poll_sleep", &g_poll_sleep, MIN0},
  {"persistent_spin", &g_persistent_spin, MIN0},
  {"ln_bwd4", &g_ln_bwd4, AS_GIVEN},
  {"mel_exact_log", &g_mel_exact_log, AS_GIVEN},
  {"text_emit", &g_text_emit, AS_GIVEN},
  {"text_passes", &g_text_passes, AS_GIVEN},
};
}

extern "C" int zeggs_set_option(const char* name, int value) {
  for (const Option& o : k_options) {
    if (strcmp(name, o.name) != 0) continue;
    if (o.kind == CALL) return o.set(value);
    const int lo = o.kind == MIN1 ? 1 : 0;
    *o.target = o.kind == AS_GIVEN ? value : o.kind == NONZERO ? value != 0 : value < lo ? lo : value;
    return 0;
  }
  zeggs_set_error("unknown option %s", name);
  return -1;
}
```

### ubisoft-laforge-zeroeggs_amd/zeggs/capi.py

```python
import ctypes as C
import os
import threading
from pathlib import Path

LIB_PATH = Path(os.environ.get("ZEGGS_LIB") or Path(__file__).resolve().parent / "libzeggs_hip.so")
OPTIONS = {}


class HipLibraryMissing(RuntimeError):
    pass


def _struct(name, fields):
    return type(name, (C.Structure,), {"_fields_": [(f, t) for t, names in fields for f in names.split()]})


def _ptr_struct(name, fields):
    return type(name, (C.Structure,), {"_fields_": [(f, C.c_void_p) for f in fields]})


SpeechDims = _struct("SpeechDims", [(C.c_int, "B T F H O KW"), (C.c_float, "dropout_p"), (C.c_uint64, "seed")])
LiveDims = _struct("LiveDims", [(C.c_int, "R F H O KW D feat_ld out_ld")])
LiveRow = _struct("LiveRow", [(C.c_long, "n_ring k0 last"), (C.c_int, "n_new n_out feat_off reserved")])
StyleDims = _struct("StyleDims", [(C.c_int, "B L C H E NH dropout"), (C.c_uint64, "seed")])
# ... 51 lines not shown
    "zeggs_speech_encoder_live_workspace_bytes": "size_t: ZeggsLiveDims*",
    "zeggs_speech_encoder_live_prepare": "status: ZeggsLiveDims* ZeggsSpeechParams* any* size_t stream",
    "zeggs_speech_encoder_live": "status: ZeggsLiveDims* ZeggsSpeechParams* f32* f32* ZeggsLiveRow* f32* f32* f32* any* size_t stream",
    "zeggs_style_encoder_workspace_bytes": "size_t: ZeggsStyleDims*",
    "zeggs_style_encoder_fwd": "status: ZeggsStyleDims* ZeggsStyleParams* f32* f32* f32* any* size_t stream",
    "zeggs_style_encoder_fwd_part": "status: ZeggsStyleDims* ZeggsStyleParams* f32* f32* f32* any* size_t stream int",
    "zeggs_style_encoder_input_offset": "size_t: ZeggsStyleDims*",
    "zeggs_style_encoder_bwd": "status: ZeggsStyleDims* ZeggsStyleParams* f32* ZeggsStyleGrads* any* size_t stream",
    "zeggs_style_encoder_bwd_ex": "status: ZeggsStyleDims* ZeggsStyleParams* f32* ZeggsStyleGrads* any* size_t stream int",
    "zeggs_style_encoder_bwd_part": "status: ZeggsStyleDims* ZeggsStyleParams* f32* ZeggsStyleGrads* any* size_t stream int int",
    "zeggs_style_encoder_gru_workspace_bytes": "size_t: ZeggsStyleGruDims*",
    "zeggs_style_encoder_gru_fwd": "status: ZeggsStyleGruDims* ZeggsStyleGruParams* f32* f32* any* size_t stream",
    "zeggs_style_encoder_gru_bwd": "status: ZeggsStyleGruDims* ZeggsStyleGruParams* f32* ZeggsStyleGruGrads* any* size_t stream",
    "zeggs_vae_reparam_fwd": "status: f32* f32* f32* f32* f32* int int float stream",
    "zeggs_vae_reparam_bwd": "status: f32* f32* f32* f32* f32* f32* int int float stream",
    "zeggs_decoder_workspace_bytes": "size_t: ZeggsDecDims* int",
    "zeggs_decoder_fwd": "status: ZeggsDecDims* ZeggsDecParams* ZeggsDecStats* f32* f32* f32* f32* f32* f32* f32* f32* f32* int any* "
                         "size_t stream",
    "zeggs_decoder_fwd_state": "status: ZeggsDecDims* ZeggsDecParams* ZeggsDecStats* f32* f32* f32* f32* f32* f32* f32* f32* f32* f32* "
                               "f32* any* size_t stream",
    "zeggs_persistent_state": "int: int",
    "zeggs_tp_stamps": "status: ZeggsDecDims* any* size_t host*",
    "zeggs_tp_waits": "status: ZeggsDecDims* any* size_t host*",
    "zeggs_tp_dual_stamps": "status: ZeggsDecDims* any* size_t host*",
    "zeggs_bp_stamps": "status: ZeggsDecDims* any* size_t host*",
    "zeggs_bp_waits": "status: ZeggsDecDims* any* size_t host*",
    "zeggs_decoder_chain_errors": "status: ZeggsDecDims* int any* size_t host*",
    "zeggs_decoder_chain_stamps": "status: ZeggsDecDims* int any* size_t host*",
    "zeggs_decoder_bwd": "status: ZeggsDecDims* ZeggsDecParams* ZeggsDecStats* f32* f32* f32* f32* f32* f32* f32* ZeggsDecGrads* f32* "
                         "f32* any* size_t stream",
    "zeggs_decoder_fwd_ex": "status: ZeggsDecDims* ZeggsDecParams* ZeggsDecStats* f32* f32* f32* f32* f32* f32* f32* f32* f32* int any* "
                            "size_t stream ZeggsDecCall*",
    "zeggs_decoder_bwd_ex": "status: ZeggsDecDims* ZeggsDecParams* ZeggsDecStats* f32* f32* f32* f32* f32* f32* f32* ZeggsDecGrads* f32* "
                            "f32* any* size_t stream ZeggsDecCall*",
    "zeggs_decoder_fwd_state_ex": "status: ZeggsDecDims* ZeggsDecParams* ZeggsDecStats* f32* f32* f32* f32* f32* f32* f32* f32* f32* "
                                  "f32* f32* any* size_t stream ZeggsDecCall*",
    "zeggs_decoder_batch_workspace_bytes": "size_t: ZeggsDecDims*",
    "zeggs_decoder_batch_prepare": "mask: ZeggsDecDims* ZeggsDecParams* ZeggsDecStats* any* size_t stream",
    "zeggs_decoder_state_init": "status: ZeggsDecDims* ZeggsDecParams* ZeggsDecStats* f32* f32* f32* f32* f32* f32* any* size_t stream",
    "zeggs_decoder_fwd_batch": "status: ZeggsDecDims* ZeggsDecParams* ZeggsDecStats* f32* f32* f32* f32* f32* f32* f32* f32* f32* f32* "
                               "f32* any* size_t stream ZeggsDecCall* int",
    "zeggs_decoder_batch_last_path": "int:",
    "zeggs_decoder_wgrads": "status: ZeggsDecDims* ZeggsDecGrads* any* size_t int stream",
    "zeggs_decoder_prepare": "mask: ZeggsDecDims* ZeggsDecParams* ZeggsDecStats* any* size_t stream",
    "zeggs_side_stream": "status: host*",
    "zeggs_loss_workspace_bytes": "size_t: ZeggsLossDims*",
    "zeggs_loss_fwd_bwd": "status: ZeggsLossDims* i32* f32* f32* f32* f32* f32* f32* f32* f32* f32* float f32* f32* f32* f32* f32* f32* "
                          "float any* size_t stream",
    "zeggs_loss_prepare_truth": "status: ZeggsLossDims* i32* f32* f32* f32* f32* any* size_t stream",
    "zeggs_loss_fwd_bwd_ex": "status: ZeggsLossDims* i32* f32* f32* f32* f32* f32* f32* f32* f32* f32* float f32* f32* f32* f32* f32* "
                             "f32* float any* size_t stream int",
    "zeggs_loss_eval_workspace_bytes": "size_t: ZeggsLossDims*",
    "zeggs_loss_eval": "status: ZeggsLossDims* i32* f32* f32* f32* f32* f32* f32* f32* f32* f32* f64* any* size_t stream",
    "zeggs_eval_accumulate": "status: f64* i32* int int f64* stream",
    "zeggs_gemm_fixed_order": "int: int",
    "zeggs_test_gemm_route_log": "int: int host* host* int",
    "zeggs_radam_step": "status: f32* f32* f32* f32* long float float float float int stream",
    "zeggs_radam_step_guarded": "status: f32* f32* f32* f32* long float float float float int i32* f32* stream",
    "zeggs_radam_step_guarded_part": "status: f32* f32* f32* f32* long float float float float int i32* f32* int stream",
    "zeggs_radam_step_wd": "status: f32* f32* f32* f32* long float float float float int float i32* f32* int stream",
    "zeggs_radam_step_c": "status: f32* f32* f32* f32* long float float float float float float int float i32* f32* int stream",
    "zeggs_radam_step_d": "status: f32* f32* f32* f32* long double double double double float float int float i32* f32* int stream",
    "zeggs_status_flag": "status: i32* f32* stream",
    "zeggs_test_cotenant": "status: int int float f32* long stream",
    "zeggs_test_attention_fwd": "status: f32* f32* f32* int int int int float uint64 stream",
    "zeggs_test_attention_bwd": "status: f32* f32* f32* f32* f32* f32* f32* int int int int float uint64 stream",
    "zeggs_gather_windows": "status: f32* int i64* int int f32* stream",
    "zeggs_gather_rows": "status: f32* int i64* long f32* int stream",
    "zeggs_mel_stft_frames": "long: ZeggsMelDims* long",
    "zeggs_mel_workspace_bytes": "size_t: ZeggsMelDims* long",
    "zeggs_mel_features": "status: ZeggsMelDims* f32* long f64* int f32* any* size_t stream",
    "zeggs_mel_frames_ready": "long: ZeggsMelDims* long",
    "zeggs_mel_range_workspace_bytes": "size_t: ZeggsMelDims* long long",
    "zeggs_mel_features_range": "status: ZeggsMelDims* f32* long int f64* long long f32* any* size_t stream",
    "zeggs_mel_window_first_sample": "long: ZeggsMelDims* long",
    "zeggs_mel_features_window": "status: ZeggsMelDims* f32* long long int f64* long long f32* any* size_t stream",
    "zeggs_mel_last_form": "int:",
    "zeggs_loudness_workspace_bytes": "size_t: long int long",
    "zeggs_loudness_gain": "status: f32* long int double host* host* long i64* i64* int int f64* f32* any* size_t stream",
    "zeggs_gather_example": "status: f32* int i64* int int f32* f32* f32* int int stream",
    "zeggs_normalize_rows": "status: f32* long int long f32* f32* float stream",
    "zeggs_fill": "status: f32* long float stream",
    "zeggs_scale_copy": "status: f32* f32* long f32* float stream",
    "zeggs_randn": "status: f32* long uint64 stream",
    "zeggs_dropout": "status: f32* long float uint64 stream",
    "zeggs_broadcast_time": "status: f32* f32* int int int stream",
    "zeggs_sum_time": "status: f32* f32* int int int stream",
    "zeggs_normalize_vec_fwd": "status: f32* f32* long int float stream",
    "zeggs_normalize_vec_bwd": "status: f32* f32* f32* long int float stream",
    "zeggs_vectorize_input_fwd": "status: int int f32* f32* f32* f32* f32* f32* f32* f32* f32* f32* f32* f32* stream",
    "zeggs_vectorize_input_bwd": "status: int int f32* f32* f32* f32* f32* f32* f32* f32* f32* f32* f32* f32* f32* f32* stream",
    "zeggs_devectorize_output_fwd": "status: int int float f32* f32* f32* f32* f32* f32* f32* f32* stream",
    "zeggs_devectorize_output_bwd": "status: int int float f32* f32* f32* f32* f32* f32* f32* f32* f32* f32* f32* stream",
    "zeggs_kl_div_fwd": "status: f32* f32* int int f32* stream",
    "zeggs_kl_div_bwd": "status: f32* f32* int int f32* f32* f32* stream",
    "zeggs_mask_from_lengths": "status: i64* int int u8* stream",
    "zeggs_anim_features_workspace_bytes": "size_t: ZeggsAnimDims*",
    "zeggs_anim_features": "status: ZeggsAnimDims* i32* f64* f64* ZeggsAnimOut* any* size_t stream",
    "zeggs_pose_to_bvh": "status: ZeggsBvhDims* f32* f32* f32* f32* f64* f64* stream",
    "zeggs_pose_to_bvh_table": "status: ZeggsBvhDims* f32* f32* f32* f32* f32* f32* i32* f64* stream",
    "zeggs_write_table_text": "status: str int host* long int",
    "zeggs_parse_table_text": "status: host* size_t host* long int",
    "zeggs_format_table_text": "status: host* long int host* size_t host*",
    "zeggs_table_text_workspace_bytes": "size_t: long int",
    "zeggs_table_text_device": "status: f64* long int u8* size_t i64* i32* any* size_t stream",
    "zeggs_spline_chunk": "status: host* host* host*",
    "zeggs_spline_resample_workspace_bytes": "size_t: long int",
    "zeggs_spline_resample": "status: f64* long int long f64* any* size_t stream",
    "zeggs_rot_stretch_workspace_bytes": "size_t: long int long",
    "zeggs_rot_stretch": "status: f64* long int long int f64* any* size_t stream",
    "zeggs_audio_prepare": "status: f32* long i64* int long long f32* f64* stream",
    "zeggs_center_take": "status: f64* f64* long int int int any* size_t stream",
    "zeggs_masked_stats_workspace_bytes": "size_t: long int",
    "zeggs_masked_stats": "status: f32* u8* long int f64* f64* f64* any* size_t stream",
    "zeggs_sweep_graph_stats": "status: host* host*",
}

MelRow = _struct("MelRow", [(C.c_void_p, "wav out"), (C.c_long, "base n_samples k0 k1"), (C.c_int, "final")])
Seg = _struct("Seg", [(C.c_void_p, "src dst"), (C.c_long, "count")])
EXT_STRUCTS = {"ZeggsMelRow": MelRow, "ZeggsSeg": Seg}
EXT_PROTOTYPES = {
    "zeggs_mel_batch_tables_bytes": "size_t: ZeggsMelDims*",
    "zeggs_mel_batch_prepare": "status: ZeggsMelDims* f64* any* size_t stream",
    "zeggs_mel_batch_workspace_bytes": "size_t: ZeggsMelDims* int long",
    "zeggs_mel_features_batch": "status: ZeggsMelDims* ZeggsMelRow* ZeggsMelRow* int f64* any* any* size_t stream",
    "zeggs_mel_batch_last_ops": "int:",
    "zeggs_copy_segments": "status: ZeggsSeg* ZeggsSeg* int stream",
}

LoudDims = _struct("LoudDims", [(C.c_int, "fs rows ring_blocks warmup"), (C.c_double, "target gain_lo gain_hi"), (C.c_double * 10, "coef")])
LoudRow = _struct("LoudRow", [(C.c_void_p, "src dst"), (C.c_long, "count"), (C.c_int, "row")])
LOUD_STRUCTS = {"ZeggsLoudDims": LoudDims, "ZeggsLoudRow": LoudRow}
LOUD_PROTOTYPES = {
    "zeggs_live_loudness_state_bytes": "size_t: ZeggsLoudDims*",
    "zeggs_live_loudness_reset": "status: ZeggsLoudDims* any* size_t int float stream",
    "zeggs_live_loudness_hold": "status: ZeggsLoudDims* any* size_t int int stream",
    "zeggs_live_loudness_push": "status: ZeggsLoudDims* ZeggsLoudRow* ZeggsLoudRow* int any* size_t stream",
    "zeggs_live_loudness_read": "status: ZeggsLoudDims* any* size_t int host* stream",
}

ResampleDims = _struct("ResampleDims", [(C.c_int, "rows history")])
ResampleRow = _struct("ResampleRow", [(C.c_void_p, "src dst table"), (C.c_long, "count n_in n_out outputs WL"),
                                      (C.c_int, "row format final L M")])
RS_STRUCTS = {"ZeggsResampleDims": ResampleDims, "ZeggsResampleRow": ResampleRow}
RS_PROTOTYPES = {
    "zeggs_live_resample_version": "int:",
    "zeggs_resample_state_bytes": "size_t: ZeggsResampleDims*",
    "zeggs_resample_reset": "status: ZeggsResampleDims* any* size_t int stream",
    "zeggs_resample_push": "status: ZeggsResampleDims* ZeggsResampleRow* ZeggsResampleRow* int any* size_t stream",
    "zeggs_resample_flush": "status: ZeggsResampleDims* ZeggsResampleRow* any* size_t stream",
    "zeggs_resample_whole": "status: f64* int int long any* int long f32* long stream",
}


class DevicePointer(C.c_void_p):
    dtypes = None
    _ok = None

    @classmethod
    def from_param(cls, t):
        if t is None:
            return None
        try:
            on_gpu = t.is_cuda
        except AttributeError:
            if isinstance(t, (int, C.c_void_p)):
                return C.c_void_p.from_param(t)
            raise TypeError(f"zeggs: a tensor, None or an address where the library reads a device pointer, not {type(t).__name__}") from None
        if not on_gpu:
            raise RuntimeError("zeggs: tensor is not on a GPU (the HIP engine has no CPU path)")
        if cls.dtypes is not None:
            if cls._ok is None:
                import torch
                cls._ok = tuple(getattr(torch, n) for n in cls.dtypes)
            if t.dtype not in cls._ok:
                raise TypeError(f"zeggs: {t.dtype} tensor where the library reads {' / '.join(cls.dtypes)}")
        if not t.is_contiguous():
            raise RuntimeError("zeggs: tensor must be contiguous")
        return C.c_void_p(t.data_ptr())


def _device_pointer(name, dtypes):
    return type(name, (DevicePointer,), {"dtypes": dtypes})


KINDS = {"int": C.c_int, "long": C.c_long, "size_t": C.c_size_t, "uint64": C.c_uint64, "float": C.c_float, "double": C.c_double,
         "str": C.c_char_p, "host*": C.c_void_p, "stream": C.c_void_p,
         "f32*": _device_pointer("f32_p", ("float32",)), "f64*": _device_pointer("f64_p", ("float64",)),
         "i32*": _device_pointer("i32_p", ("int32",)), "i64*": _device_pointer("i64_p", ("int64",)),
         "u8*": _device_pointer("u8_p", ("uint8", "bool")), "any*": _device_pointer("any_p", None)}
KINDS.update({name + "*": C.POINTER(cls) for name, cls in {**STRUCTS, **EXT_STRUCTS, **LOUD_STRUCTS, **RS_STRUCTS}.items()})
RETURNS = {"status": C.c_int, "mask": C.c_int, "int": C.c_int, "long": C.c_long, "size_t": C.c_size_t, "str": C.c_char_p}


def signature(name):
    ret, _, params = (PROTOTYPES.get(name) or EXT_PROTOTYPES.get(name) or LOUD_PROTOTYPES.get(name) or RS_PROTOTYPES[name]).partition(":")
    return ret, params.split()


class _Typed(C.CDLL):

    def __init__(self, path):
        super().__init__(path)
        base = self._FuncPtr

        class _Fn(base):
            _flags_, _restype_ = base._flags_, base._restype_

            def __call__(self, *args, _call=base.__call__):
                try:
                    return _call(self, *args)
                except C.ArgumentError as e:
                    raise (TypeError if ": TypeError: " in str(e) else RuntimeError)(f"{self.__name__}: {e}") from None
        self._FuncPtr = _Fn


_HANDLES = None
_LOCK = threading.Lock()


def _load():
    global _HANDLES
    with _LOCK:
        if _HANDLES is not None:
            return _HANDLES
        if not LIB_PATH.exists():
            raise HipLibraryMissing(
                f"{LIB_PATH} not found: build it with `python -c 'import __graft_entry__ as g; g.build()'` "
                "(hipcc --offload-arch=gfx950). The ZeroEGGS MI355X engine has no CPU fallback.")
        typed, plain = _Typed(str(LIB_PATH)), C.CDLL(str(LIB_PATH))
        missing = [n for n in (*PROTOTYPES, *EXT_PROTOTYPES, *LOUD_PROTOTYPES, *RS_PROTOTYPES) if not hasattr(plain, n)]
        if missing:
            raise HipLibraryMissing(f"{LIB_PATH} is older than this package (no {', '.join(missing)}): rebuild it")
        last_error = typed.zeggs_last_error

        def status(rc, fn, args):
            if rc != 0:
                raise RuntimeError(f"{fn.__name__}: {last_error().decode()}")
            return rc

        def mask(rc, fn, args):
            return rc if rc >= 0 else status(rc, fn, args)
        for name in (*PROTOTYPES, *EXT_PROTOTYPES, *LOUD_PROTOTYPES, *RS_PROTOTYPES):
            ret, params = signature(name)
            fn = getattr(typed, name)
            fn.argtypes, fn.restype = [KINDS[k] for k in params], RETURNS[ret]
            if ret in ("status", "mask"):
                fn.errcheck = status if ret == "status" else mask
            getattr(plain, name).restype = RETURNS[ret]
        for kv in filter(None, os.environ.get("ZEGGS_OPTIONS", "").split(",")):
            k, v = kv.split("=")
            try:
                typed.zeggs_set_option(k.strip().encode(), int(v))
            except RuntimeError as e:
                raise RuntimeError(f"ZEGGS_OPTIONS: {str(e).partition(': ')[2]}") from None
            OPTIONS[k.strip()] = int(v)
        _HANDLES = (typed, plain)
        return _HANDLES


def api():
    return (_HANDLES or _load())[0]


def raw():
    return (_HANDLES or _load())[1]
```

### ubisoft-laforge-zeroeggs_amd/zeggs/ops.py

```python
import ctypes as C

import numpy as np
import torch

from . import capi
from .capi import (DEC_FIELDS, SPEECH_FIELDS, STATS_FIELDS, STYLE_FIELDS, STYLE_GRU_FIELDS, DecCall, DecDims, DecPtrs,
                   DecStats, HipLibraryMissing, LiveDims, LiveRow, LossDims, LoudDims, LoudRow, MelRow, ResampleDims, ResampleRow,
                   Seg, SpeechDims, SpeechPtrs,
                   StyleDims, StyleGruDims, StyleGruPtrs, StylePtrs, api)

_LIB_PATH = capi.LIB_PATH

COUNTERS = {}
STATUS_WORDS = 4
GAVE_UP = {1: "B=1 decode kernel", 2: "training rollout", 4: "BPTT sweep", 8: "batch decode sweep"}


def lib():
    return capi.raw()


def _check(rc, what):
    if rc != 0:
        raise RuntimeError(f"{what}: {lib().zeggs_last_error().decode()}")
# ... 959 lines not shown
        predicted, root_pos, root_rot, out_mean, out_std = (_f32c(t) for t in (predicted, root_pos, root_rot, out_mean,
                                                                                 out_std))
        B = predicted.shape[0]
        dev = predicted.device
        pose = torch.empty(B, 6 + 15 * J, device=dev, dtype=torch.float32)
        nrp = torch.empty(B, 3, device=dev, dtype=torch.float32)
        nrr = torch.empty(B, 4, device=dev, dtype=torch.float32)
        api().zeggs_devectorize_output_fwd(B, J, dt, predicted, root_pos, root_rot, out_mean, out_std, pose, nrp, nrr, _stream())
        ctx.save_for_backward(predicted, root_pos, root_rot, out_mean, out_std)
        ctx.dims = (B, J, dt)
        ctx.set_materialize_grads(False)
        return pose, nrp, nrr

    @staticmethod
    def backward(ctx, dpose, dnrp, dnrr):
        predicted, root_pos, root_rot, out_mean, out_std = ctx.saved_tensors
        B, J, dt = ctx.dims
        c = lambda g: _f32c(g) if g is not None else None
        dpred, drp, drr = torch.empty_like(predicted), torch.empty_like(root_pos), torch.empty_like(root_rot)
        api().zeggs_devectorize_output_bwd(B, J, dt, predicted, root_pos, root_rot, out_mean, out_std, c(dpose), c(dnrp), c(dnrr),
                                           dpred, drp, drr, _stream())
        return dpred, drp, drr, None, None, None, None


def devectorize_output(predicted, root_pos, root_rot, njoints, dt, out_mean, out_std):
    return _DevectorizeFn.apply(predicted, root_pos, root_rot, int(njoints), float(dt), out_mean, out_std)


class _KLFn(torch.autograd.Function):
    @staticmethod
    def forward(ctx, mu, logvar):
        mu, logvar = _f32c(mu), _f32c(logvar)
        out = torch.empty((), device=mu.device, dtype=torch.float32)
        api().zeggs_kl_div_fwd(mu, logvar, mu.shape[0], mu.numel() // mu.shape[0], out, _stream())
        ctx.save_for_backward(mu, logvar)
        return out

    @staticmethod
    def backward(ctx, dout):
        mu, logvar = ctx.saved_tensors
        dmu, dlv = torch.empty_like(mu), torch.empty_like(logvar)
        api().zeggs_kl_div_bwd(mu, logvar, mu.shape[0], mu.numel() // mu.shape[0], _f32c(dout).reshape(1), dmu, dlv, _stream())
        return dmu, dlv


def kl_div(mu, logvar):
    return _KLFn.apply(mu, logvar)


def mask_from_lengths(lengths):
    lengths = lengths.to(torch.int64).contiguous()
    B = lengths.shape[0]
    max_len = int(lengths.max().item())
    mask = torch.empty(B, max_len, device=lengths.device, dtype=torch.uint8)
    api().zeggs_mask_from_lengths(lengths, B, max_len, mask, _stream())
    return mask.view(torch.bool)


class _LossFn(torch.autograd.Function):
    @staticmethod
    def forward(ctx, o_pose, o_rpos, o_rrot, mu, logvar, w_pose, w_rpos, w_rrot, gaze, parents, kl_weight, dt, gscale,
                unit_grad, truth_ws):
        o_pose, o_rpos, o_rrot, w_pose, w_rpos, w_rrot, gaze = (
            _f32c(t) for t in (o_pose, o_rpos, o_rrot, w_pose, w_rpos, w_rrot, gaze))
        B, T, PO = o_pose.shape
        J = (PO - 6) // 15
        has_kl = mu is not None and kl_weight > 0
        S = mu.shape[1] if mu is not None else 0
        d = LossDims(B, T, J, S, float(dt))
        L = api()
        dev = o_pose.device
        need = L.zeggs_loss_workspace_bytes(d)
        prepared = truth_ws is not None and truth_ws.numel() >= need
        ws = truth_ws if prepared else _ws(need, dev)
        terms = torch.empty(19, device=dev, dtype=torch.float32)
        dpose, drpos, drrot = torch.empty_like(o_pose), torch.empty_like(o_rpos), torch.empty_like(o_rrot)
        dmu = torch.empty(B, S, device=dev) if mu is not None else None
        dlv = torch.empty(B, S, device=dev) if mu is not None else None
        L.zeggs_loss_fwd_bwd_ex(d, parents, o_pose, o_rpos, o_rrot, w_pose, w_rpos, w_rrot, gaze,
                                _f32c(mu) if mu is not None else None, _f32c(logvar) if mu is not None else None,
                                kl_weight if has_kl else 0.0, terms, dpose, drpos, drrot, dmu, dlv, gscale, ws, ws.numel(), _stream(),
                                int(prepared))
        ctx.save_for_backward(dpose, drpos, drrot, dmu, dlv)
        ctx.unit_grad = bool(unit_grad)
        ctx.mark_non_differentiable(terms)
        ctx.set_materialize_grads(False)
        loss = torch.empty((), device=dev, dtype=torch.float32)
        scale_copy(terms[18:19], out=loss)
        return loss, terms

    @staticmethod
    def backward(ctx, g, _gterms):
        dpose, drpos, drrot, dmu, dlv = ctx.saved_tensors
        if g is None:
            return (None,) * 15
        if not ctx.unit_grad:
            g = _f32c(g).reshape(1)
            dpose, drpos, drrot = scale_copy(dpose, g), scale_copy(drpos, g), scale_copy(drrot, g)
            if dmu is not None:
                dmu, dlv = scale_copy(dmu, g), scale_copy(dlv, g)
        return (dpose, drpos, drrot, dmu, dlv, None, None, None, None, None, None, None, None, None, None)


def loss_prepare_truth(w_pose, w_rpos, w_rrot, gaze, parents, dt, ws=None):
    w_pose, w_rpos, w_rrot, gaze = (_f32c(t) for t in (w_pose, w_rpos, w_rrot, gaze))
    B, T, PO = w_pose.shape
    d = LossDims(B, T, (PO - 6) // 15, 0, float(dt))
    L = api()
    need = int(L.zeggs_loss_workspace_bytes(d))
    if ws is None or ws.numel() != need or ws.device != w_pose.device:
        ws = _ws(need, w_pose.device)
    L.zeggs_loss_prepare_truth(d, parents, w_pose, w_rpos, w_rrot, gaze, ws, ws.numel(), _stream())
    return ws


def training_loss(o_pose, o_rpos, o_rrot, w_pose, w_rpos, w_rrot, gaze, parents, dt, mu=None, logvar=None,
                  kl_weight=0.0, gscale=1.0, unit_grad=False, truth_ws=None):
    return _LossFn.apply(o_pose, o_rpos, o_rrot, mu, logvar, w_pose, w_rpos, w_rrot, gaze, parents,
                         float(kl_weight), float(dt), float(gscale), bool(unit_grad), truth_ws)


EVAL_COLS = 22


def loss_eval(o_pose, o_rpos, o_rrot, w_pose, w_rpos, w_rrot, gaze, parents, dt, mu=None, logvar=None, rows=None, ws=None):
    o_pose, o_rpos, o_rrot, w_pose, w_rpos, w_rrot, gaze = (_f32c(t) for t in (o_pose, o_rpos, o_rrot, w_pose, w_rpos, w_rrot, gaze))
    B, T, PO = o_pose.shape
    S = mu.shape[1] if mu is not None else 0
    d = LossDims(B, T, (PO - 6) // 15, S, float(dt))
    L = api()
    dev = o_pose.device
    need = int(L.zeggs_loss_eval_workspace_bytes(d))
    if ws is None or ws.numel() < need or ws.device != dev:
        ws = _ws(need, dev)
    if rows is None or tuple(rows.shape) != (B, EVAL_COLS) or rows.device != dev:
        rows = torch.empty(B, EVAL_COLS, device=dev, dtype=torch.float64)
    L.zeggs_loss_eval(d, parents, o_pose, o_rpos, o_rrot, w_pose, w_rpos, w_rrot, gaze, _f32c(mu) if mu is not None else None,
                      _f32c(logvar) if mu is not None else None, rows, ws, ws.numel(), _stream())
    return rows


class fixed_order_gemms:

    def __enter__(self):
        self.prev = api().zeggs_gemm_fixed_order(1)

    def __exit__(self, *exc):
        api().zeggs_gemm_fixed_order(int(self.prev))
        return False


GEMM_ROUTES = ("none", "skinny", "m32-split", "m32", "mid-split", "streamk-direct", "streamk-bf16-split", "streamk-dma",
               "streamk-lds-128x128", "streamk-lds-256x128", "splitk", "half", "tile-128x128", "tile-64x64")
GEMM_SPLITTING_ROUTES = ("m32-split", "mid-split", "streamk-direct", "streamk-bf16-split", "streamk-dma", "streamk-lds-128x128",
                         "streamk-lds-256x128", "splitk")


def gemm_route_log(reset=False):
    last, counts = (C.c_int * 4)(), (C.c_long * len(GEMM_ROUTES))()
    n = api().zeggs_test_gemm_route_log(int(bool(reset)), last, counts, len(GEMM_ROUTES))
    if n != len(GEMM_ROUTES):
        raise RuntimeError(f"zeggs.ops.GEMM_ROUTES names {len(GEMM_ROUTES)} routes, the library has {n}: rebuild it")
    return {"route": GEMM_ROUTES[last[0]], "splitk": int(last[1]), "tile": (int(last[2]), int(last[3])),
            "counts": {GEMM_ROUTES[i]: int(c) for i, c in enumerate(counts) if c}}


def loss_eval_workspace(B, T, J, S, dt, device):
    d = LossDims(int(B), int(T), int(J), int(S), float(dt))
    return _ws(api().zeggs_loss_eval_workspace_bytes(d), device)


def eval_accumulate(rows, group, acc):
    B, groups = rows.shape[0], acc.shape[0]
    assert rows.shape == (B, EVAL_COLS) and acc.shape == (groups, EVAL_COLS + 1) and group.shape == (B,)
    api().zeggs_eval_accumulate(rows, group, int(B), int(groups), acc, _stream())
    return acc


def radam_step(p, g, m, v, beta1, beta2, eps, step_scale, rectified, status=None, gflag=None, count=True, decay=0.0):
    api().zeggs_radam_step_d(p, g, m, v, p.numel(), beta1, beta2, 1 - beta1, 1 - beta2, eps, step_scale, int(rectified), decay, status,
                             gflag if status is not None else None, int(bool(count)), _stream())


def status_flag(status, dst):
    api().zeggs_status_flag(status, dst, _stream())


def gather_windows(frames, starts, T, out=None):
    B, W = starts.shape[0], frames.shape[1]
    if out is None or out.shape != (B, T, W) or not out.is_contiguous():
        out = torch.empty(B, T, W, device=frames.device, dtype=torch.float32)
    api().zeggs_gather_windows(frames, W, starts, B, T, out, _stream())
    return out


def gather_rows(frames, rows, out=None, out_ld=None):
    W = frames.shape[1]
    n = rows.numel()
    if out is None:
        out = torch.empty(*rows.shape, W, device=frames.device, dtype=torch.float32)
        out_ld = W
    api().zeggs_gather_rows(frames, W, rows.contiguous(), n, out, int(out_ld), _stream())
    return out


def normalize_rows_(x, mean, std):
    W = x.shape[-1]
    rows = x.numel() // W
    vec = std if torch.is_tensor(std) and std.dim() > 0 else None
    sc = 1.0 if vec is not None else float(std)
    api().zeggs_normalize_rows(x, rows, W, W, mean, vec, sc, _stream())
    return x


_OPTIONS = capi.OPTIONS
_PERSISTENT_OPTION = ("persistent", "train_persistent", "bwd_persistent")


def _persistent_live(which):
    return _OPTIONS.get(_PERSISTENT_OPTION[which], 1) != 0 and api().zeggs_persistent_state(which) == 1


def set_option(name, value):
    global _CHAIN_DIAGNOSTICS, _LAST_DECODER_WS
    api().zeggs_set_option(name.encode(), int(value))
    _OPTIONS[name] = int(value)
    if name == "chain":
        _CHAIN_DIAGNOSTICS = bool(value)
        if not value:
            _LAST_DECODER_WS = None
```

Baseline: 494,400 frames/s.

## Group style-encoder weight-gradient GEMMs into one split-K grouped TN launch

Adds a grouped TN GEMM kernel that runs a table of up to 16 problems in a single launch. Each problem is split along K so the total workgroup count targets two per CU, and results accumulate atomically into zeroed outputs. The style encoder backward now batches the ff2, ff0, out, in and c4 weight gradients (conv taps written straight into the strided dW layout, with no unpack) into one launch placed after the c4 stage, instead of several GEMM and unpack launches. This trades launch overhead and under-filled small GEMMs for atomic accumulation, an extra zero-fill pass and nondeterministic summation order.

```diff
diff --git a/include/zeggs_hip.h b/include/zeggs_hip.h
--- a/include/zeggs_hip.h
+++ b/include/zeggs_hip.h
@@ -244,6 +244,7 @@
   ZEGGS_GEMM_ROUTE_HALF,
   ZEGGS_GEMM_ROUTE_TILE_128,
   ZEGGS_GEMM_ROUTE_TILE_64,
+  ZEGGS_GEMM_ROUTE_GROUPED_TN,
   ZEGGS_GEMM_ROUTE_COUNT
 };
 int zeggs_test_gemm_route_log(int reset, int* last4, long* counts, int ncounts);
diff --git a/include/zeggs_hip_gemm.h b/include/zeggs_hip_gemm.h
--- /dev/null
+++ b/include/zeggs_hip_gemm.h
@@ -0,0 +1,28 @@
+#ifndef ZEGGS_HIP_GEMM_H
+#define ZEGGS_HIP_GEMM_H
+#include "zeggs_hip.h"
+
+#ifdef __cplusplus
+extern "C" {
+#endif
+
+#define ZEGGS_TN_GROUP_MAX 16
+
+typedef struct {
+  const float* A;
+  const float* B;
+  float* C;
+  int M, N, K;
+  int kbatch;
+  long sak, sbk;
+  long kbsA, kbsB;
+  long scm, scn;
+  float beta;
+} ZeggsTnProblem;
+
+int zeggs_gemm_tn_grouped(const ZeggsTnProblem* table, int n, void* stream);
+
+#ifdef __cplusplus
+}
+#endif
+#endif
diff --git a/ubisoft-laforge-zeroeggs_amd/csrc/encoders.hip b/ubisoft-laforge-zeroeggs_amd/csrc/encoders.hip
--- a/ubisoft-laforge-zeroeggs_amd/csrc/encoders.hip
+++ b/ubisoft-laforge-zeroeggs_amd/csrc/encoders.hip
@@ -306,6 +306,7 @@
                                           const ZeggsStyleGrads* G, void* ws, size_t ws_bytes, void* stream, int grads_zeroed) {
   return zeggs_style_encoder_bwd_part(dp, P, dout, G, ws, ws_bytes, stream, grads_zeroed, 3);
 }
+int g_style_wgrads_grouped = 1;
 extern "C" int zeggs_style_encoder_bwd_part(const ZeggsStyleDims* dp, const ZeggsStyleParams* P, const float* dout,
                                             const ZeggsStyleGrads* G, void* ws, size_t ws_bytes, void* stream, int grads_zeroed,
                                             int part) {
@@ -322,26 +323,55 @@
   const float p2 = d.dropout ? 0.2f : 0.f, p1 = d.dropout ? 0.1f : 0.f;
   float *t0 = w.t0, *t1 = w.t1, *t2 = w.t2, *t3 = w.t3;
   float *t0a = w.t0a, *t0b = w.t0b, *t1a = w.t1a;
+  const bool acc = grads_zeroed != 0;
   auto dw_ff2 = [&](hipStream_t q) -> int {
     ZTRY(conv_dw_gemm(w.f1p, (long)LP * E, E, t0a + E, E, (long)LP * E, w.dwf, 3 * E, E, B, L, q));
-    return k_unpack_conv_dw(G->ff2_w, w.dwf, E, E, 3, q);
+    return k_unpack_conv_dw(G->ff2_w, w.dwf, E, E, 3, q, acc);
   };
   auto dw_ff0 = [&](hipStream_t q) -> int {
     ZTRY(conv_dw_gemm(w.ap, (long)LP * E, E, t0b + E, E, (long)LP * E, w.dwf, 3 * E, E, B, L, q));
-    return k_unpack_conv_dw(G->ff0_w, w.dwf, E, E, 3, q);
+    return k_unpack_conv_dw(G->ff0_w, w.dwf, E, E, 3, q, acc);
   };
   auto dw_out = [&](hipStream_t q) -> int { return gemm_tn(t1a, E, w.O, E, G->out_w, E, (int)BL, E, E, gb, q); };
   auto dw_in = [&](hipStream_t q) -> int { return gemm_tn(w.dqkv, 3 * E, w.h, E, G->in_w, E, (int)BL, 3 * E, E, gb, q); };
   auto dw_c4 = [&](hipStream_t q) -> int {
     ZTRY(conv_dw_gemm(w.a1p, (long)LP * H, H, t0 + E, E, (long)LP * E, w.dwf, 3 * H, E, B, L, q));
-    return k_unpack_conv_dw(G->c4_w, w.dwf, E, H, 3, q);
+    return k_unpack_conv_dw(G->c4_w, w.dwf, E, H, 3, q, acc);
   };
   auto dw_c0 = [&](hipStream_t q) -> int {
     ZTRY(conv_dw_gemm(w.xp, (long)LP * C, C, t2, H, (long)L * H, w.dwf, 3 * C, H, B, L, q));
-    return k_unpack_conv_dw(G->c0_w, w.dwf, H, C, 3, q);
+    return k_unpack_conv_dw(G->c0_w, w.dwf, H, C, 3, q, acc);
+  };
+  const bool grouped = g_style_wgrads_grouped && !gemm_fixed_order();
+  auto dw_small = [&](hipStream_t q) -> int {
+    ZeggsTnProblem pr[11];
+    memset(pr, 0, sizeof(pr));
+    int n = 0;
+    auto conv = [&](const float* xp, int Ci, const float* dyp, float* dW) {
+      for (int tap = 0; tap < 3; ++tap) {
+        ZeggsTnProblem& p = pr[n++];
+        p.A = dyp + E; p.B = xp + (long)tap * Ci; p.C = dW + tap;
+        p.M = E; p.N = Ci; p.K = L; p.kbatch = B;
+        p.sak = E; p.sbk = Ci; p.kbsA = (long)LP * E; p.kbsB = (long)LP * Ci; p.scm = 3L * Ci; p.scn = 3; p.beta = gb;
+      }
+    };
+    auto linear = [&](const float* dy, int N, const float* x, float* dW) {
+      ZeggsTnProblem& p = pr[n++];
+      p.A = dy; p.B = x; p.C = dW;
+      p.M = N; p.N = E; p.K = (int)BL; p.kbatch = 1;
+      p.sak = N; p.sbk = E; p.scm = E; p.scn = 1; p.beta = gb;
+    };
+    conv(w.f1p, E, t0a, G->ff2_w);
+    conv(w.ap, E, t0b, G->ff0_w);
+    linear(t1a, E, w.O, G->out_w);
+    linear(w.dqkv, 3 * E, w.h, G->in_w);
+    conv(w.a1p, H, t0, G->c4_w);
+    return gemm_tn_grouped(pr, n, q);
   };
   if (only_w) {
-    ZTRY(dw_ff2(s)); ZTRY(dw_ff0(s)); ZTRY(dw_out(s)); ZTRY(dw_in(s)); ZTRY(dw_c4(s)); ZTRY(dw_c0(s));
+    if (grouped) ZTRY(dw_small(s));
+    else { ZTRY(dw_ff2(s)); ZTRY(dw_ff0(s)); ZTRY(dw_out(s)); ZTRY(dw_in(s)); ZTRY(dw_c4(s)); }
+    ZTRY(dw_c0(s));
     return 0;
   }
   (void)chain;
@@ -363,14 +393,14 @@
     q.dx_raw = rv(t2); q.out = t0ain; q.pad_L = L; q.p_post = p1; q.seed_post = d.seed + 5; q.dbias = G->ff2_b;
     ZTRY(k_ln_bwd_fused(q, s));
   }
-  if (inl) ZTRY(dw_ff2(s));
+  if (inl && !grouped) ZTRY(dw_ff2(s));
   ZTRY(conv_gemm(t0a, (long)LP * E, E, w.wfb2, 3 * E, E, t1, E, (long)L * E, nullptr, B, L, ACT_NONE, s));
   {
     LnBwdFused q = ln_bwd_fused_args((int)BL, E);
     q.dyA = rv(t1); q.out = t0bin; q.pad_L = L; q.ysave = rv(w.f1p + E, L, (long)LP * E); q.act = ACT_RELU; q.dbias = G->ff0_b;
     ZTRY(k_ln_bwd_fused(q, s));
   }
-  if (inl) ZTRY(dw_ff0(s));
+  if (inl && !grouped) ZTRY(dw_ff0(s));
   ZTRY(conv_gemm(t0b, (long)LP * E, E, w.wfb0, 3 * E, E, t1, E, (long)L * E, nullptr, B, L, ACT_NONE, s));
   {
     LnBwdFused q = ln_bwd_fused_args((int)BL, E);
@@ -379,7 +409,7 @@
     q.dx_raw = rv(t3); q.out = rv(t1a); q.p_post = p1; q.seed_post = d.seed + 4; q.dbias = G->out_b;
     ZTRY(k_ln_bwd_fused(q, s));
   }
-  if (inl) ZTRY(dw_out(s));
+  if (inl && !grouped) ZTRY(dw_out(s));
   ZTRY(gemm_nn(t1a, E, P->out_w, E, t2, E, (int)BL, E, E, 0.f, s));
   if (w.fused) {
     ZTRY(k_attn_bwd(w.qkv, w.O, w.lse, t2, w.dqkv, w.dsum, G->in_b, B, L, E, NH, p1, d.seed + 3, s));
@@ -416,7 +446,7 @@
     ZTRY(launch_gemm(g, B * NH, s));
   }
   }
-  if (inl) ZTRY(dw_in(s));
+  if (inl && !grouped) ZTRY(dw_in(s));
   if (!w.fused) ZTRY(k_colsum(G->in_b, w.dqkv, BL, 3 * E, 3 * E, gb, s));
   ZTRY(gemm_nn(w.dqkv, 3 * E, P->in_w, E, t1, E, (int)BL, 3 * E, E, 0.f, s));
   {
@@ -426,7 +456,7 @@
     q.out = t0in; q.pad_L = L; q.ysave = rv(w.c2, L, (long)LP * E); q.act = ACT_RELU; q.dbias = G->c4_b;
     ZTRY(k_ln_bwd_fused(q, s));
   }
-  if (inl) ZTRY(dw_c4(s));
+  if (inl) ZTRY(grouped ? dw_small(s) : dw_c4(s));
   ZTRY(conv_gemm(t0, (long)LP * E, E, w.wb4, 3 * E, H, t1, H, (long)L * H, nullptr, B, L, ACT_NONE, s));
   {
     LnBwdFused q = ln_bwd_fused_args((int)BL, H);
diff --git a/ubisoft-laforge-zeroeggs_amd/csrc/gemm.h b/ubisoft-laforge-zeroeggs_amd/csrc/gemm.h
--- a/ubisoft-laforge-zeroeggs_amd/csrc/gemm.h
+++ b/ubisoft-laforge-zeroeggs_amd/csrc/gemm.h
@@ -1,5 +1,7 @@
 #pragma once
 #include <hip/hip_runtime.h>
+
+#include "../../include/zeggs_hip_gemm.h"
 
 struct GemmArgs {
   const float* A;
@@ -32,3 +34,5 @@
             int K, float beta, hipStream_t s);
 int gemm_tn_bias(const float* dy, long lddy, const float* x, long ldx, float* dW, long lddw, int M_contract, int N,
                  int K, float beta, float* db, hipStream_t s);
+int gemm_tn_grouped(const ZeggsTnProblem* problems, int n, hipStream_t s);
+bool gemm_fixed_order();
diff --git a/ubisoft-laforge-zeroeggs_amd/csrc/gemm.hip b/ubisoft-laforge-zeroeggs_amd/csrc/gemm.hip
--- a/ubisoft-laforge-zeroeggs_amd/csrc/gemm.hip
+++ b/ubisoft-laforge-zeroeggs_amd/csrc/gemm.hip
@@ -570,7 +570,7 @@
 }
 
 enum GemmRoute { GR_NONE = 0, GR_SKINNY, GR_M32_SPLIT, GR_M32, GR_MID_SPLIT, GR_SK_DIRECT, GR_SK_BF16_SPLIT, GR_SK_DMA, GR_SK_LDS_128,
-                 GR_SK_LDS_256, GR_SPLITK, GR_HALF, GR_TILE_128, GR_TILE_64, GR_COUNT };
+                 GR_SK_LDS_256, GR_SPLITK, GR_HALF, GR_TILE_128, GR_TILE_64, GR_GROUPED_TN, GR_COUNT };
 struct GemmRouteLog { int route, splitk, bm, bn; long count[GR_COUNT]; };
 static thread_local GemmRouteLog tl_gemm_log;
 static inline void log_route(int route, int splitk, int bm, int bn) {
@@ -659,6 +659,43 @@
   return launch_streamk_cfg<128, 128, 2, 2>(g, ncu, s);
 }
 
+struct GroupRow {
+  const float *A, *B;
+  float* C;
+  long sak, sbk, kbsA, kbsB, scm, scn;
+  int M, N, K, kbatch;
+  int tx, slices, wg_end, fill;
+};
+struct GroupTable { GroupRow r[ZEGGS_TN_GROUP_MAX]; int n; };
+template <int BM, int BN, int WM, int WN>
+__global__ __launch_bounds__(WM* WN * 64, GEMM_MINB) void gemm_tn_grouped_kernel(GroupTable t) {
+  constexpr int LDA = BM + 4, LDB = BN + 4;
+  __shared__ __attribute__((aligned(16))) float As2[2][BK * LDA];
+  __shared__ __attribute__((aligned(16))) float Bs2[2][BK * LDB];
+  const int w = blockIdx.x;
+  int p = 0, first = 0;
+  while (p + 1 < t.n && w >= t.r[p].wg_end) { first = t.r[p].wg_end; ++p; }
+  const GroupRow& r = t.r[p];
+  GemmArgs g;
+  g.A = r.A; g.B = r.B; g.C = r.C; g.bias = nullptr;
+  g.M = r.M; g.N = r.N; g.K = r.K;
+  g.sam = 1; g.sak = r.sak; g.sbk = r.sbk; g.sbn = 1; g.scm = r.scm; g.scn = r.scn;
+  g.kbatch = r.kbatch; g.kbsA = r.kbsA; g.kbsB = r.kbsB;
+  g.alpha = 1.f; g.beta = 1.f; g.act = ACT_NONE;
+  const int local = w - first, tile = local / r.slices, ks = local - tile * r.slices;
+  const int by = tile / r.tx, bx = tile - by * r.tx;
+  const int ntiles_all = ((r.K + BK - 1) / BK) * r.kbatch;
+  const int t_begin = (int)((long)ntiles_all * ks / r.slices), t_end = (int)((long)ntiles_all * (ks + 1) / r.slices);
+  gemm_tile<BM, BN, WM, WN, false, false>(g, g.A, g.B, g.C, by * BM, bx * BN, t_begin, t_end, true, &As2[0][0], &Bs2[0][0]);
+}
+__global__ void gemm_tn_grouped_fill_k(GroupTable t) {
+  const GroupRow& r = t.r[blockIdx.y];
+  if (!r.fill) return;
+  const long n = (long)r.M * r.N;
+  for (long i = (long)blockIdx.x * blockDim.x + threadIdx.x; i < n; i += (long)gridDim.x * blockDim.x)
+    r.C[(i / r.N) * r.scm + (i % r.N) * r.scn] = 0.f;
+}
+
 struct SkinnyArgs {
   const float *x, *W, *bias;
   float* y;
@@ -916,6 +953,73 @@
   return launch_cfg<64, 64, 2, 2>(g, nbatch, s);
 }
 
+constexpr int GROUPED_WGS_PER_CU = 2;
+bool gemm_fixed_order() { return t_gemm_fixed_order != 0; }
+int gemm_tn_grouped(const ZeggsTnProblem* pr, int n, hipStream_t s) {
+  ZCHECK(pr != nullptr && n >= 1 && n <= ZEGGS_TN_GROUP_MAX, "gemm_tn_grouped: a table of 1 .. %d problems, not %d", ZEGGS_TN_GROUP_MAX, n);
+  for (int i = 0; i < n; ++i) {
+    const ZeggsTnProblem& p = pr[i];
+    ZCHECK(p.M >= 0 && p.N >= 0 && p.K >= 0 && p.kbatch >= 1, "gemm_tn_grouped: problem %d: M, N, K >= 0 and kbatch >= 1", i);
+    ZCHECK(p.beta == 0.f || p.beta == 1.f, "gemm_tn_grouped: problem %d: beta is 0 or 1, not %g", i, (double)p.beta);
+    ZCHECK((p.A && p.B && p.C) || p.M == 0 || p.N == 0, "gemm_tn_grouped: problem %d: null operand", i);
+    ZCHECK((long)cdiv(p.K, BK) * p.kbatch < (1L << 30), "gemm_tn_grouped: problem %d: contraction too long", i);
+  }
+  if (t_gemm_fixed_order) {
+    for (int i = 0; i < n; ++i) {
+      const ZeggsTnProblem& p = pr[i];
+      GemmArgs g = gemm_args(p.A, p.B, p.C, p.M, p.N, p.K);
+      g.sam = 1; g.sak = p.sak; g.sbk = p.sbk; g.sbn = 1; g.scm = p.scm; g.scn = p.scn;
+      g.kbatch = p.kbatch; g.kbsA = p.kbsA; g.kbsB = p.kbsB; g.beta = p.beta;
+      ZTRY(launch_gemm(g, 1, s));
+    }
+    return 0;
+  }
+  constexpr int BM = 128, BN = 128;
+  GroupTable t;
+  memset(&t, 0, sizeof(t));
+  long all_kt = 0;
+  for (int i = 0; i < n; ++i)
+    if (pr[i].M > 0 && pr[i].N > 0) all_kt += (long)cdiv(pr[i].M, BM) * cdiv(pr[i].N, BN) * cdiv(pr[i].K, BK) * pr[i].kbatch;
+  const long aim = (long)device_cus() * GROUPED_WGS_PER_CU;
+  long q = (all_kt + aim - 1) / aim;
+  if (q < 8) q = 8;
+  long wgs = 0, fill_n = 0;
+  int most = 1;
+  for (int i = 0; i < n; ++i) {
+    const ZeggsTnProblem& p = pr[i];
+    if (p.M == 0 || p.N == 0) continue;
+    GroupRow& r = t.r[t.n++];
+    r.A = p.A; r.B = p.B; r.C = p.C;
+    r.sak = p.sak; r.sbk = p.sbk; r.kbsA = p.kbsA; r.kbsB = p.kbsB; r.scm = p.scm; r.scn = p.scn;
+    r.M = p.M; r.N = p.N; r.K = p.K; r.kbatch = p.kbatch;
+    r.tx = cdiv(p.N, BN);
+    const long kt = (long)cdiv(p.K, BK) * p.kbatch;
+    long sl = (kt + q / 2) / q;
+    if (sl > kt) sl = kt;
+    if (sl < 1) sl = 1;
+    r.slices = (int)sl;
+    most = r.slices > most ? r.slices : most;
+    wgs += (long)r.tx * cdiv(p.M, BM) * sl;
+    ZCHECK(wgs < (1L << 30), "gemm_tn_grouped: too many workgroups");
+    r.wg_end = (int)wgs;
+    r.fill = p.beta == 0.f;
+    if (r.fill && (long)p.M * p.N > fill_n) fill_n = (long)p.M * p.N;
+  }
+  if (t.n == 0) return 0;
+  if (fill_n > 0) {
+    const long blocks = (fill_n + 255) / 256;
+    hipLaunchKernelGGL(gemm_tn_grouped_fill_k, dim3((unsigned)(blocks > 256 ? 256 : blocks), (unsigned)t.n), dim3(256), 0, s, t);
+    ZLAUNCH_CHECK("gemm_tn_grouped_fill");
+  }
+  log_route(GR_GROUPED_TN, most, BM, BN);
+  hipLaunchKernelGGL((gemm_tn_grouped_kernel<BM, BN, 2, 2>), dim3((unsigned)wgs), dim3(256), 0, s, t);
+  ZLAUNCH_CHECK("gemm_tn_grouped");
+  return 0;
+}
+extern "C" int zeggs_gemm_tn_grouped(const ZeggsTnProblem* table, int n, void* stream) {
+  return gemm_tn_grouped(table, n, (hipStream_t)stream);
+}
+
 extern "C" int zeggs_test_gemm_route_log(int reset, int* last4, long* counts, int ncounts) {
   if (last4) { last4[0] = tl_gemm_log.route; last4[1] = tl_gemm_log.splitk; last4[2] = tl_gemm_log.bm; last4[3] = tl_gemm_log.bn; }
   for (int i = 0; counts && i < ncounts; ++i) counts[i] = i < GR_COUNT ? tl_gemm_log.count[i] : 0;
diff --git a/ubisoft-laforge-zeroeggs_amd/csrc/kernels.h b/ubisoft-laforge-zeroeggs_amd/csrc/kernels.h
--- a/ubisoft-laforge-zeroeggs_amd/csrc/kernels.h
+++ b/ubisoft-laforge-zeroeggs_amd/csrc/kernels.h
@@ -64,7 +64,7 @@
 int k_pack_conv_w(float* wf, float* wb, const float* w, int Co, int Ci, int Kw, hipStream_t s);
 struct PackConvW { float *wf, *wb; const float* w; int Co, Ci, Kw; };
 int k_pack_conv_w_multi(const PackConvW* items, int n, hipStream_t s);
-int k_unpack_conv_dw(float* dw, const float* dwf, int Co, int Ci, int Kw, hipStream_t s);
+int k_unpack_conv_dw(float* dw, const float* dwf, int Co, int Ci, int Kw, hipStream_t s, bool accumulate = false);
 int k_add_rows_bcast(float* h, const float* table, int B, int L, int C, hipStream_t s);
 int k_meanpool_fwd(float* out, const float* f, int B, int L, int C, hipStream_t s);
 int k_meanpool_bwd(float* df, const float* dout, int B, int L, int C, hipStream_t s);
diff --git a/ubisoft-laforge-zeroeggs_amd/csrc/kernels.hip b/ubisoft-laforge-zeroeggs_amd/csrc/kernels.hip
--- a/ubisoft-laforge-zeroeggs_amd/csrc/kernels.hip
+++ b/ubisoft-laforge-zeroeggs_amd/csrc/kernels.hip
@@ -614,6 +614,7 @@
   }
 }
 
+template <bool ACC>
 __global__ __launch_bounds__(256) void unpack_conv_dw_t_k(float* dw, const float* dwf, int Co, int Ci, int Kw) {
   __shared__ float t[4][32][33];
   const int ci0 = blockIdx.x * 32, co0 = blockIdx.y * 32, tx = threadIdx.x & 31, ty = threadIdx.x >> 5;
@@ -629,18 +630,23 @@
     if (co >= Co) continue;
     for (int e = tx; e < run; e += 32) {
       const int cl = e / Kw, j = e - cl * Kw, ci = ci0 + cl;
-      if (ci < Ci) dw[((long)co * Ci + ci) * Kw + j] = t[j][cl][r];
-    }
-  }
-}
-
+      if (ci < Ci) {
+        float* o = dw + ((long)co * Ci + ci) * Kw + j;
+        *o = ACC ? *o + t[j][cl][r] : t[j][cl][r];
+      }
+    }
+  }
+}
+
+template <bool ACC>
 __global__ void unpack_conv_dw_k(float* dw, const float* dwf, int Co, int Ci, int Kw) {
   long n = (long)Co * Ci * Kw;
   GS_LOOP(i, n) {
     int j = (int)(i % Kw);
     long r = i / Kw;
     int ci = (int)(r % Ci), co = (int)(r / Ci);
-    dw[i] = dwf[((long)j * Ci + ci) * Co + co];
+    const float v = dwf[((long)j * Ci + ci) * Co + co];
+    dw[i] = ACC ? dw[i] + v : v;
   }
 }
 
@@ -861,14 +867,17 @@
   L1D(pack_conv_w_multi_k, tot, s, q);
   return 0;
 }
-int k_unpack_conv_dw(float* dw, const float* dwf, int Co, int Ci, int Kw, hipStream_t s) {
+int k_unpack_conv_dw(float* dw, const float* dwf, int Co, int Ci, int Kw, hipStream_t s, bool accumulate) {
   long n = (long)Co * Ci * Kw;
   if (Kw <= 4 && n >= 65536) {
-    hipLaunchKernelGGL(unpack_conv_dw_t_k, dim3(cdiv(Ci, 32), cdiv(Co, 32)), dim3(256), 0, s, dw, dwf, Co, Ci, Kw);
+    const dim3 grid(cdiv(Ci, 32), cdiv(Co, 32));
+    if (accumulate) hipLaunchKernelGGL(unpack_conv_dw_t_k<true>, grid, dim3(256), 0, s, dw, dwf, Co, Ci, Kw);
+    else hipLaunchKernelGGL(unpack_conv_dw_t_k<false>, grid, dim3(256), 0, s, dw, dwf, Co, Ci, Kw);
     ZLAUNCH_CHECK("unpack_conv_dw_t");
     return 0;
   }
-  L1D(unpack_conv_dw_k, n, s, dw, dwf, Co, Ci, Kw);
+  if (accumulate) L1D(unpack_conv_dw_k<true>, n, s, dw, dwf, Co, Ci, Kw);
+  else L1D(unpack_conv_dw_k<false>, n, s, dw, dwf, Co, Ci, Kw);
   return 0;
 }
 int k_add_rows_bcast(float* h, const float* table, int B, int L, int C, hipStream_t s) {
diff --git a/ubisoft-laforge-zeroeggs_amd/csrc/options.hip b/ubisoft-laforge-zeroeggs_amd/csrc/options.hip
--- a/ubisoft-laforge-zeroeggs_amd/csrc/options.hip
+++ b/ubisoft-laforge-zeroeggs_amd/csrc/options.hip
@@ -7,6 +7,7 @@
 extern int g_stage_variant, g_timing, g_chain, g_sweep_graphs, g_launch_window;
 extern int g_tp_tiles4, g_tp_dual;
 extern int g_gemm_wg_target, g_gemm_streamk_wgs, g_gemm_mid_split, g_gemm_skinny, g_gemm_streamk, g_gemm_split_bf16;
+extern int g_style_wgrads_grouped;
 extern int g_text_emit, g_text_passes;
 extern int g_mel_mfma, g_mel_fft, g_mel_exact_log, g_loss_lds, g_ln_bwd4;
 void zeggs_gemm_set_dma(int on), zeggs_gemm_set_direct(int mode, int wgs), zeggs_gemm_set_direct_depth(int d);
@@ -48,6 +49,7 @@
   {"gemm_asum", nullptr, CALL, [](int v) { zeggs_gemm_set_asum(v); return 0; }},
   {"gemm_skinny", &g_gemm_skinny, NONZERO},
   {"gemm_streamk", &g_gemm_streamk, NONZERO},
+  {"style_wgrads_grouped", &g_style_wgrads_grouped, NONZERO},
   {"fused_attention", &g_fused_attention, NONZERO},
   {"bwd_chunks", &g_bwd_chunks, MIN1},
   {"tp_tiles4", &g_tp_tiles4, NONZERO},
diff --git a/ubisoft-laforge-zeroeggs_amd/zeggs/capi.py b/ubisoft-laforge-zeroeggs_amd/zeggs/capi.py
--- a/ubisoft-laforge-zeroeggs_amd/zeggs/capi.py
+++ b/ubisoft-laforge-zeroeggs_amd/zeggs/capi.py
@@ -227,6 +227,13 @@
     "zeggs_resample_whole": "status: f64* int int long any* int long f32* long stream",
 }
 
+TnProblem = _struct("TnProblem", [(C.c_void_p, "A B C"), (C.c_int, "M N K kbatch"), (C.c_long, "sak sbk kbsA kbsB scm scn"),
+                                  (C.c_float, "beta")])
+GG_STRUCTS = {"ZeggsTnProblem": TnProblem}
+GG_PROTOTYPES = {
+    "zeggs_gemm_tn_grouped": "status: ZeggsTnProblem* int stream",
+}
+
 
 class DevicePointer(C.c_void_p):
     dtypes = None
@@ -264,12 +271,13 @@
          "f32*": _device_pointer("f32_p", ("float32",)), "f64*": _device_pointer("f64_p", ("float64",)),
          "i32*": _device_pointer("i32_p", ("int32",)), "i64*": _device_pointer("i64_p", ("int64",)),
          "u8*": _device_pointer("u8_p", ("uint8", "bool")), "any*": _device_pointer("any_p", None)}
-KINDS.update({name + "*": C.POINTER(cls) for name, cls in {**STRUCTS, **EXT_STRUCTS, **LOUD_STRUCTS, **RS_STRUCTS}.items()})
+KINDS.update({name + "*": C.POINTER(cls) for name, cls in {**STRUCTS, **EXT_STRUCTS, **LOUD_STRUCTS, **RS_STRUCTS, **GG_STRUCTS}.items()})
 RETURNS = {"status": C.c_int, "mask": C.c_int, "int": C.c_int, "long": C.c_long, "size_t": C.c_size_t, "str": C.c_char_p}
 
 
 def signature(name):
-    ret, _, params = (PROTOTYPES.get(name) or EXT_PROTOTYPES.get(name) or LOUD_PROTOTYPES.get(name) or RS_PROTOTYPES[name]).partition(":")
+    ret, _, params = (PROTOTYPES.get(name) or EXT_PROTOTYPES.get(name) or LOUD_PROTOTYPES.get(name) or RS_PROTOTYPES.get(name) or
+                       GG_PROTOTYPES[name]).partition(":")
     return ret, params.split()
 
 
@@ -304,7 +312,7 @@
                 f"{LIB_PATH} not found: build it with `python -c 'import __graft_entry__ as g; g.build()'` "
                 "(hipcc --offload-arch=gfx950). The ZeroEGGS MI355X engine has no CPU fallback.")
         typed, plain = _Typed(str(LIB_PATH)), C.CDLL(str(LIB_PATH))
-        missing = [n for n in (*PROTOTYPES, *EXT_PROTOTYPES, *LOUD_PROTOTYPES, *RS_PROTOTYPES) if not hasattr(plain, n)]
+        missing = [n for n in (*PROTOTYPES, *EXT_PROTOTYPES, *LOUD_PROTOTYPES, *RS_PROTOTYPES, *GG_PROTOTYPES) if not hasattr(plain, n)]
         if missing:
             raise HipLibraryMissing(f"{LIB_PATH} is older than this package (no {', '.join(missing)}): rebuild it")
         last_error = typed.zeggs_last_error
@@ -316,7 +324,7 @@
 
         def mask(rc, fn, args):
             return rc if rc >= 0 else status(rc, fn, args)
-        for name in (*PROTOTYPES, *EXT_PROTOTYPES, *LOUD_PROTOTYPES, *RS_PROTOTYPES):
+        for name in (*PROTOTYPES, *EXT_PROTOTYPES, *LOUD_PROTOTYPES, *RS_PROTOTYPES, *GG_PROTOTYPES):
             ret, params = signature(name)
             fn = getattr(typed, name)
             fn.argtypes, fn.restype = [KINDS[k] for k in params], RETURNS[ret]
diff --git a/ubisoft-laforge-zeroeggs_amd/zeggs/ops.py b/ubisoft-laforge-zeroeggs_amd/zeggs/ops.py
--- a/ubisoft-laforge-zeroeggs_amd/zeggs/ops.py
+++ b/ubisoft-laforge-zeroeggs_amd/zeggs/ops.py
@@ -1135,17 +1135,32 @@
 
 GEMM_ROUTES = ("none", "skinny", "m32-split", "m32", "mid-split", "streamk-direct", "streamk-bf16-split", "streamk-dma",
                "streamk-lds-128x128", "streamk-lds-256x128", "splitk", "half", "tile-128x128", "tile-64x64")
+GEMM_GROUPED_ROUTES = ("grouped-tn",)
 GEMM_SPLITTING_ROUTES = ("m32-split", "mid-split", "streamk-direct", "streamk-bf16-split", "streamk-dma", "streamk-lds-128x128",
-                         "streamk-lds-256x128", "splitk")
+                         "streamk-lds-256x128", "splitk", "grouped-tn")
+_ROUTE_NAMES = GEMM_ROUTES + GEMM_GROUPED_ROUTES
 
 
 def gemm_route_log(reset=False):
-    last, counts = (C.c_int * 4)(), (C.c_long * len(GEMM_ROUTES))()
-    n = api().zeggs_test_gemm_route_log(int(bool(reset)), last, counts, len(GEMM_ROUTES))
-    if n != len(GEMM_ROUTES):
-        raise RuntimeError(f"zeggs.ops.GEMM_ROUTES names {len(GEMM_ROUTES)} routes, the library has {n}: rebuild it")
-    return {"route": GEMM_ROUTES[last[0]], "splitk": int(last[1]), "tile": (int(last[2]), int(last[3])),
-            "counts": {GEMM_ROUTES[i]: int(c) for i, c in enumerate(counts) if c}}
+    last, counts = (C.c_int * 4)(), (C.c_long * len(_ROUTE_NAMES))()
+    n = api().zeggs_test_gemm_route_log(int(bool(reset)), last, counts, len(_ROUTE_NAMES))
+    if n != len(_ROUTE_NAMES):
+        raise RuntimeError(f"zeggs.ops names {len(_ROUTE_NAMES)} GEMM routes, the library has {n}: rebuild it")
+    return {"route": _ROUTE_NAMES[last[0]], "splitk": int(last[1]), "tile": (int(last[2]), int(last[3])),
+            "counts": {_ROUTE_NAMES[i]: int(c) for i, c in enumerate(counts) if c}}
+
+
+def gemm_tn_grouped(problems):
+    table = (capi.TnProblem * len(problems))()
+    for row, p in zip(table, problems):
+        for t in (p["A"], p["B"], p["C"]):
+            if not (t.is_cuda and t.dtype == torch.float32 and t.is_contiguous()):
+                raise TypeError("zeggs.ops.gemm_tn_grouped: contiguous float32 tensors on the device")
+        row.A, row.B, row.C = p["A"].data_ptr(), p["B"].data_ptr(), p["C"].data_ptr()
+        row.M, row.N, row.K, row.kbatch = int(p["M"]), int(p["N"]), int(p["K"]), int(p.get("kbatch", 1))
+        row.sak, row.sbk, row.kbsA, row.kbsB = int(p["sak"]), int(p["sbk"]), int(p.get("kbsA", 0)), int(p.get("kbsB", 0))
+        row.scm, row.scn, row.beta = int(p["scm"]), int(p["scn"]), float(p.get("beta", 0.0))
+    api().zeggs_gemm_tn_grouped(table, len(problems), _stream())
 
 
 def loss_eval_workspace(B, T, J, S, dt, device):
```

Result: no change. 496,500 frames/s, median of 6 (+0.4%).
